# ralexstokes/ethereum_consensus

Hardware: NVIDIA H100
Metric: fast_aggregate_verify tuples/s (higher is better)
Workload: dtype u32 limbs (381-bit Fp), u32 SHA-256 words

## Files before the change

ethereum_consensus_b200/build.py:

```python
from __future__ import annotations

import os
import subprocess
import sys
from concurrent.futures import ThreadPoolExecutor
from pathlib import Path

PKG = Path(__file__).resolve().parent
CSRC = PKG / "csrc"
LIB = PKG / "libb200_consensus.so"
OBJ = PKG / "build"
NVCC = os.environ.get("NVCC", "/usr/local/cuda/bin/nvcc")
ARCH = ["-gencode", "arch=compute_90a,code=sm_90a"]
FLAGS = [*ARCH, "-lineinfo", "-O3", "-std=c++17",
         "-Xcompiler", "-fPIC,-fvisibility=hidden", "--expt-relaxed-constexpr"]
DEFAULT_PTXAS_OPT = {"bls_g1.cu": 2, "bls_g2.cu": 1, "bls_vm.cu": 1}


def _stale(target: Path, deps) -> bool:
    if not target.exists():
        return True
    t = target.stat().st_mtime
    return any(Path(d).stat().st_mtime > t for d in deps)


def build(force: bool = False, verbose: bool = False, defines=(), suffix: str = "", ptxas_opt=None) -> Path:
    global LIB, OBJ
    env_opt = {kv.split(":")[0]: int(kv.split(":")[1]) for kv in os.environ.get("B200_PTXAS_OPT", "").split(",") if kv}
    ptxas_opt = {**DEFAULT_PTXAS_OPT, **env_opt, **dict(ptxas_opt or {})}
    if suffix:
        LIB = PKG / f"libb200_consensus{suffix}.so"
        OBJ = PKG / f"build{suffix}"
    srcs = sorted(CSRC.glob("*.cu"))
    hdrs = sorted(CSRC.glob("*.cuh")) + sorted(CSRC.glob("*.h")) + sorted((PKG.parent / "include").glob("*.h"))
    OBJ.mkdir(exist_ok=True)
    jobs = []
    def command(s, o):
        cmd = [NVCC, *FLAGS, *[f"-D{d}" for d in defines], "-c", str(s), "-o", str(o)]
        if s.name in ptxas_opt and int(ptxas_opt[s.name]) != 3:
            cmd[1:1] = ["-Xptxas", f"-O{int(ptxas_opt[s.name])}"]
        return cmd

    for s in srcs:
        o = OBJ / (s.stem + ".o")
        stamp = o.with_suffix(".cmd")
        if force or _stale(o, [s] + hdrs) or not stamp.exists() or stamp.read_text() != " ".join(command(s, o)):
            jobs.append((s, o))

    def cc(job):
        s, o = job
        cmd = command(s, o)
        stamp = o.with_suffix(".cmd")
        if verbose:
            cmd.insert(1, "-Xptxas=-v")
        r = subprocess.run(cmd, capture_output=True, text=True)
        if r.returncode != 0:
            raise RuntimeError(f"nvcc failed for {s.name}:\n{r.stdout}\n{r.stderr}")
        stamp.write_text(" ".join(command(s, o)))
        return r.stderr

    with ThreadPoolExecutor(max_workers=min(8, max(1, len(jobs)))) as ex:
        for msg in ex.map(cc, jobs):
            if verbose and msg:
                print(msg, file=sys.stderr)
    objs = [OBJ / (s.stem + ".o") for s in srcs]
    if force or jobs or _stale(LIB, objs):
        cmd = [NVCC, "-shared", "-o", str(LIB), *map(str, objs), *ARCH,
               "-Xcompiler", "-fPIC", "-cudart", "static"]
        r = subprocess.run(cmd, capture_output=True, text=True)
        if r.returncode != 0:
            raise RuntimeError(f"link failed:\n{r.stdout}\n{r.stderr}")
    return LIB


if __name__ == "__main__":
    defs = [a[2:] for a in sys.argv[1:] if a.startswith("-D")]
    suf = next((a.split("=", 1)[1] for a in sys.argv[1:] if a.startswith("--suffix=")), "")
    popt = next((a.split("=", 1)[1] for a in sys.argv[1:] if a.startswith("--ptxas-opt=")), "")
    popt = {kv.split(":")[0]: int(kv.split(":")[1]) for kv in popt.split(",") if kv}
    print(build(force="--force" in sys.argv, verbose="-v" in sys.argv, defines=defs, suffix=suf, ptxas_opt=popt))
```

ethereum_consensus_b200/csrc/bls_kernels.cuh:

```cuda
#pragma once
#include <cstddef>
#include <cstdint>

#include "groups.cuh"
#include "fp12.cuh"

namespace b200 {

struct G1Pre {
    Fp xz, y, z3;
    uint32_t inf;
};

enum : uint32_t { TUPLE_FLAG_EMPTY = 1u, TUPLE_FLAG_AGG_INF = 2u };
enum : int32_t { SIG_OK = 0, SIG_NOT_IN_GROUP = -1 };

void set_g1_variant(int v);
void set_g1_small_n(uint32_t n);
void set_small_cta(int threads);
void set_vm_team16_max(uint32_t n);
void set_vm_cta(int threads);
void launch_g1_validate(const uint8_t* keys, uint32_t n, G1Aff* out, int32_t* codes, void* stream, int cta = 0);
void launch_g1_aggregate(const G1Aff* keys, const int32_t* key_codes, const uint32_t* index, const uint32_t* off,
                         uint32_t n_tuples, G1Aff* agg, G1Pre* agg_pre, int32_t* pk_code, uint32_t* flags,
                         uint32_t extra_flags, void* stream, G1Jac* agg_jac = nullptr);
void launch_rlc_scale(const G1Jac* agg, const G2Aff* sig, const int32_t* pk_code, const uint32_t* flags, const int32_t* sig_code,
                      const uint32_t* seed_words, uint64_t t0, uint32_t n, G1Pre* out_g1, G2Jac* out_g2, int32_t* bad, void* stream);
uint32_t launch_rlc_reduce(const Fp12* f_in, const G2Jac* q_in, uint32_t n, Fp12* f_out, G2Jac* q_out, void* stream);
void launch_rlc_finish(const G2Jac* q, G2Aff* out, void* stream);
void launch_fp12_one(Fp12* out, void* stream);
void launch_g2_sig_decode(const uint8_t* sigs, uint32_t n, G2Aff* out, int32_t* sig_code, void* stream);
void launch_hash_to_g2(const uint8_t* msgs, const uint32_t* moff, uint32_t n, G2Aff* out, void* tmp_jac, void* stream);
void launch_miller(const G1Aff* g1, const uint32_t* g1_idx, const G2Aff* g2, const uint32_t* g2_idx,
                   const uint32_t* pair_tuple, const int32_t* pk_code, const uint32_t* flags, const int32_t* sig_code,
                   uint32_t n_pairs, Fp12* f, void* stream);
void launch_final(const Fp12* f, const uint32_t* pair_off, const int32_t* pk_code, const uint32_t* flags,
                  const int32_t* sig_code, uint32_t n_tuples, int32_t* out_codes, void* stream);
int vm_init(void* stream);
int vm_load_programs(const uint32_t* blob, size_t n_words, void* stream);
void launch_vm_miller(const G1Pre* g1, const uint32_t* g1_idx, const G2Aff* g2, const uint32_t* g2_idx,
                      const uint32_t* pair_tuple, const int32_t* pk_code, const uint32_t* flags, const int32_t* sig_code,
                      uint32_t n_pairs, Fp12* f, void* stream);
void launch_vm_final(const Fp12* f, const uint32_t* pair_off, const int32_t* pk_code, const uint32_t* flags,
                     const int32_t* sig_code, uint32_t n_tuples, int32_t* out_codes, void* stream);
void launch_g2_sum_compress(const G2Aff* sigs, const int32_t* sig_code, uint32_t n, uint8_t* out96, int32_t* out_code, void* stream);
void launch_g1_compress(const G1Aff* p, uint8_t* out48, void* stream);
void launch_neg_g1(G1Aff* out, G1Pre* out_pre, void* stream);
void launch_fp_selftest(uint32_t n, uint32_t seed, uint32_t* out_mismatch, void* stream);
enum : int32_t {
    FP_EVAL_MUL = 0, FP_EVAL_SQR = 1, FPL_EVAL_MUL = 2, FPL_EVAL_SQR = 3,
    FP_EVAL_ADD = 4, FP_EVAL_SUB = 5, FP_EVAL_NEG = 6, FPL_EVAL_ADD = 7, FPL_EVAL_SUB = 8, FPL_EVAL_NEG = 9,
    FP_EVAL_ADD_RAW = 10, FP_EVAL_SUB_RAW = 11, FP_EVAL_INV_KALISKI = 12, FP_EVAL_INV_FERMAT = 13,
    FP_EVAL_SQRT = 14, FPL_EVAL_POW_SQRT = 15, FP_EVAL_IS_LEX_LARGEST = 16,
    FP_EVAL_N_OPS = 17,
    FPL_EVAL_SQRT_CHAIN = 18,
    FPL_EVAL_MUL_SUB_MUL = 19, FPL_EVAL_MUL_SUB_8SQR = 20,
    FPL_EVAL_END = 21,
    FP2_EVAL_MUL = 32, FP2_EVAL_SQR = 33, FP2_EVAL_INV = 34, FP2_EVAL_SQRT = 35, FP2_EVAL_SGN0 = 36,
    FP2_EVAL_END = 37
};
constexpr uint32_t kFpEvalIn = 24, kFpEvalOut = 25;
void launch_fp_eval(int32_t op, uint32_t n, const uint32_t* a, const uint32_t* b, uint32_t* out, void* stream);
void launch_fp2_eval(int32_t op, uint32_t n, const uint32_t* a, const uint32_t* b, uint32_t* out, void* stream);
enum : int32_t {
    CURVE_G1L_ADD_MIXED = 0, CURVE_G1L_ADD = 1, CURVE_G1L_IN_SUBGROUP = 2,
    CURVE_G1_N_OPS = 3,
    CURVE_G1L_DOUBLE = 4,
    CURVE_G2_ADD = 32, CURVE_G2_ADD_MIXED = 33, CURVE_G2_DOUBLE = 34, CURVE_G2_IN_SUBGROUP = 35, CURVE_G2_PSI = 36,
    CURVE_G2_CLEAR_COFACTOR = 37, CURVE_G2_SSWU_ISO = 38, CURVE_G2_H2C_FINISH = 39,
    CURVE_G2_END = 40
};
constexpr uint32_t kCurveEvalWords = 73;
void launch_curve_eval(int32_t op, uint32_t n, const uint32_t* a, const uint32_t* b, uint32_t* out, void* stream);
void launch_curve2_eval(int32_t op, uint32_t n, const uint32_t* a, const uint32_t* b, uint32_t* out, void* stream);
enum : int32_t {
    PAIRING_EVAL_FP6_MUL = 0, PAIRING_EVAL_FP6_INV = 1, PAIRING_EVAL_FP12_MUL = 2, PAIRING_EVAL_FP12_SQR = 3,
    PAIRING_EVAL_FP12_INV = 4, PAIRING_EVAL_FP12_MUL_BY_LINE = 5, PAIRING_EVAL_FP12_FROB1 = 6, PAIRING_EVAL_FP12_FROB2 = 7,
    PAIRING_EVAL_FP12_CYCLO_SQR = 8, PAIRING_EVAL_FP12_POW_Z = 9,
    PAIRING_EVAL_MILLER_DOUBLE = 10, PAIRING_EVAL_MILLER_ADD = 11,
    PAIRING_EVAL_MILLER_LOOP = 12, PAIRING_EVAL_FINAL_EXP = 13,
    PAIRING_EVAL_END = 14,
    PAIRING_EVAL_VM_MILLER8 = 32, PAIRING_EVAL_VM_MILLER16 = 33,
    PAIRING_EVAL_VM_FINAL8 = 34, PAIRING_EVAL_VM_FINAL16 = 35,
    PAIRING_EVAL_VM_END = 36,
    PAIRING_EVAL_FOLD_FP12 = 48, PAIRING_EVAL_FOLD_G2 = 49,
    PAIRING_EVAL_FOLD_END = 50
};
constexpr uint32_t kPairingEvalWords = 145;
void launch_pairing_eval(int32_t op, uint32_t n, const uint32_t* a, const uint32_t* b, uint32_t* out, void* stream);
void launch_vm_miller_team(int team, const G1Pre* g1, const uint32_t* idx, const G2Aff* g2, const uint32_t* zeros, uint32_t n,
                           Fp12* f, void* stream);
void launch_vm_final_team(int team, const Fp12* f, const uint32_t* pair_off, const uint32_t* zeros, uint32_t n, Fp12* f_out,
                          int32_t* codes, void* stream);

}
```

ethereum_consensus_b200/csrc/bls_vm.cu:

```cuda
#if defined(B200_VM_MUL_CALL)
#define B200_FP_MUL_CALL 1
#endif
#include <cuda_runtime.h>

#include <algorithm>

#include "bls_kernels.cuh"
#include "pairing_vm.cuh"

namespace b200 {
namespace {

__global__ void k_vm_consts(const uint32_t* __restrict__ plain, Fp2* __restrict__ out) {
    const int i = threadIdx.x;
    if (i < kVmConsts) {
        uint32_t l[24];
        for (int k = 0; k < 24; k++) l[k] = plain[i * 24 + k];
        Fp2 v;
        vm_const_to_mont(v, l);
        out[i] = v;
    }
}

struct VmOuts { int v[6]; };

template <int TEAM>
__device__ __forceinline__ void vm_run(const uint32_t* __restrict__ code, int n_rounds, const Fp2* __restrict__ consts,
                                       const VmRfStrided& rf, uint32_t lane, bool active) {
    uint32_t w = __ldg(code + lane);
#pragma unroll 1
    for (int r = 0; r < n_rounds; r++) {
        const uint32_t w_next = (r + 1 < n_rounds) ? __ldg(code + (r + 1) * TEAM + lane) : 0u;
        if (active && (w & 0xffu) != VM_NOP) {
            Fp2 res;
            vm_exec(w, rf, consts, res);
            rf.store((w >> 8) & 0xffu, res);
        }
        __syncwarp();
        w = w_next;
    }
}

__device__ __forceinline__ bool tuple_dead(uint32_t t, const int32_t* pk_code, const uint32_t* flags, const int32_t* sig_code) {
    return pk_code[t] != BLS_SUCCESS || flags[t] != 0 || sig_code[t] != SIG_OK;
}

template <int TEAM>
__global__ void __launch_bounds__(128) k_vm_miller(const uint32_t* __restrict__ code, const Fp2* __restrict__ consts,
                                                    const G1Pre* __restrict__ g1, const uint32_t* __restrict__ g1_idx,
                                                    const G2Aff* __restrict__ g2, const uint32_t* __restrict__ g2_idx,
                                                    const uint32_t* __restrict__ pair_tuple, const int32_t* __restrict__ pk_code,
                                                    const uint32_t* __restrict__ flags, const int32_t* __restrict__ sig_code,
                                                    uint32_t n_pairs, Fp12* __restrict__ f, int n_rounds, int n_slots, VmOuts outs6) {
    extern __shared__ uint32_t smem[];
    const uint32_t team_in_block = threadIdx.x / TEAM, lane = threadIdx.x % TEAM;
    const uint32_t i = blockIdx.x * (blockDim.x / TEAM) + team_in_block;
    VmRfStrided rf{smem + team_in_block * vm_team_words(uint32_t(n_slots))};
    bool active = i < n_pairs && !tuple_dead(pair_tuple[i], pk_code, flags, sig_code);
    bool trivial = false;
    if (active) {
        const G1Pre* p = g1 + g1_idx[i];
        const G2Aff* q = g2 + g2_idx[i];
        trivial = p->inf || q->inf;
        if (!trivial) {
            if (lane == 0) { Fp2 v; v.c0 = p->xz; v.c1 = fp_zero(); rf.store(0, v); }
            if (lane == 1) { Fp2 v; v.c0 = p->y; v.c1 = fp_zero(); rf.store(1, v); }
            if (lane == 2) { Fp2 v; v.c0 = p->z3; v.c1 = fp_zero(); rf.store(2, v); }
            if (lane == 3) rf.store(3, q->x);
            if (lane == 4) rf.store(4, q->y);
        }
    }
    __syncwarp();
    vm_run<TEAM>(code, n_rounds, consts, rf, lane, active && !trivial);
    static_assert(TEAM >= 6, "team must cover the six output coefficients");
    if (active && lane < 6) {
        Fp2 v;
        if (trivial) v = (lane == 0) ? fp2_one() : fp2_zero();
        else v = rf.load(uint32_t(outs6.v[lane]));
        Fp2* dst = reinterpret_cast<Fp2*>(f + i);
        const int tower_pos[6] = {0, 3, 1, 4, 2, 5};
        dst[tower_pos[lane]] = v;
    }
}

template <int TEAM, bool STORE = false>
__global__ void __launch_bounds__(128) k_vm_final(const uint32_t* __restrict__ code, const Fp2* __restrict__ consts,
                                                  const Fp12* __restrict__ f, const uint32_t* __restrict__ pair_off,
                                                  const int32_t* __restrict__ pk_code, const uint32_t* __restrict__ flags,
                                                  const int32_t* __restrict__ sig_code, uint32_t n_tuples,
                                                  int32_t* __restrict__ out_codes, int n_rounds, int n_slots, VmOuts outs6,
                                                  Fp12* __restrict__ f_out = nullptr) {
    extern __shared__ uint32_t smem[];
    const uint32_t team_in_block = threadIdx.x / TEAM, lane = threadIdx.x % TEAM;
    const uint32_t t = blockIdx.x * (blockDim.x / TEAM) + team_in_block;
    VmRfStrided rf{smem + team_in_block * vm_team_words(uint32_t(n_slots))};
    int32_t code_out = BLS_SUCCESS;
    bool active = false;
    if (t < n_tuples) {
        if (pk_code[t] != BLS_SUCCESS) code_out = pk_code[t];
        else if (sig_code[t] > 0) code_out = sig_code[t];
        else if (flags[t] != 0 || sig_code[t] == SIG_NOT_IN_GROUP) code_out = BLS_VERIFY_FAIL;
        else active = true;
    }
    if (active) {
        const int tower_pos[6] = {0, 3, 1, 4, 2, 5};
        for (uint32_t k = lane; k < 12; k += TEAM) {
            const Fp2* src = reinterpret_cast<const Fp2*>(f + pair_off[t] + k / 6);
            rf.store(k, src[tower_pos[k % 6]]);
        }
    }
    __syncwarp();
    vm_run<TEAM>(code, n_rounds, consts, rf, lane, active);
    if (STORE && active && lane < 6) {
        const int tower_pos[6] = {0, 3, 1, 4, 2, 5};
        reinterpret_cast<Fp2*>(f_out + t)[tower_pos[lane]] = rf.load(uint32_t(outs6.v[lane]));
    }
    if (t < n_tuples && lane == 0) {
        if (active) {
            bool one = fp2_eq(rf.load(uint32_t(outs6.v[0])), fp2_one());
#pragma unroll 1
            for (int k = 1; k < 6; k++) one = one && fp2_is_zero(rf.load(uint32_t(outs6.v[k])));
            code_out = one ? BLS_SUCCESS : BLS_VERIFY_FAIL;
        }
        out_codes[t] = code_out;
    }
}

}

struct VmProgramDev {
    uint32_t* d_code = nullptr;
    int rounds = 0, slots = 0;
    VmOuts outs{};
};
static VmProgramDev g_miller_prog[2], g_final_prog[2];
static Fp2* g_d_consts = nullptr;
static uint32_t g_team16_max = 2048;
static int g_vm_cta = 32;
void set_vm_team16_max(uint32_t n) { g_team16_max = n; }
void set_vm_cta(int threads) { if (threads == 32 || threads == 64 || threads == 128) g_vm_cta = threads; }

static int vm_set_program(VmProgramDev& p, const uint32_t* code, size_t bytes, int rounds, int slots, const int* outs, cudaStream_t st) {
    uint32_t* d = nullptr;
    if (cudaMalloc(&d, bytes) != cudaSuccess) return 1;
    if (cudaMemcpyAsync(d, code, bytes, cudaMemcpyHostToDevice, st) != cudaSuccess) return 1;
    if (cudaStreamSynchronize(st) != cudaSuccess) return 1;
    if (p.d_code) cudaFree(p.d_code);
    p.d_code = d; p.rounds = rounds; p.slots = slots;
    for (int k = 0; k < 6; k++) p.outs.v[k] = outs[k];
    return 0;
}
template <int TEAM>
static int vm_upload(int slot, cudaStream_t st) {
    typedef VmProg<TEAM> P;
    if (vm_set_program(g_miller_prog[slot], P::miller_code(), P::miller_code_bytes, P::miller_rounds, P::miller_slots, P::miller_out, st)) return 1;
    if (vm_set_program(g_final_prog[slot], P::final_code(), P::final_code_bytes, P::final_rounds, P::final_slots, P::final_out, st)) return 1;
    cudaFuncSetAttribute(k_vm_miller<TEAM>, cudaFuncAttributeMaxDynamicSharedMemorySize, kVmMaxSmemBytes);
    cudaFuncSetAttribute(k_vm_final<TEAM>, cudaFuncAttributeMaxDynamicSharedMemorySize, kVmMaxSmemBytes);
    cudaFuncSetAttribute(k_vm_final<TEAM, true>, cudaFuncAttributeMaxDynamicSharedMemorySize, kVmMaxSmemBytes);
    return 0;
}

int vm_load_programs(const uint32_t* blob, size_t n_words, void* stream) {
    if (!blob || n_words < 18 || blob[0] != kVmBlobMagic) return 1;
    const uint32_t team = blob[1], mr = blob[2], ms = blob[3], fr = blob[10], fs = blob[11];
    if (team != 8 && team != 16) return 1;
    if (!mr || !fr || mr > (1u << 20) || fr > (1u << 20) || ms < 12 || fs < 12 || ms > 255 || fs > 255) return 1;
    if (n_words != 18 + size_t(mr) * team + size_t(fr) * team) return 1;
    if (size_t(32 / team) * vm_team_words(std::max(ms, fs)) * 4 > size_t(kVmMaxSmemBytes)) return 1;
    auto check = [&](const uint32_t* code, uint32_t rounds, uint32_t slots, const uint32_t* outs) {
        for (int k = 0; k < 6; k++) if (outs[k] >= slots) return false;
        for (size_t i = 0; i < size_t(rounds) * team; i++) {
            const uint32_t w = code[i], op = w & 0xffu, d = (w >> 8) & 0xffu, a = (w >> 16) & 0xffu, b = w >> 24;
            if (op > VM_LDC) return false;
            if (op == VM_NOP) continue;
            if (d >= slots) return false;
            if (op == VM_LDC) { if (a >= uint32_t(kVmConsts)) return false; continue; }
            if (a >= slots) return false;
            const bool binary = op == VM_MUL || op == VM_MULFP || op == VM_ADD || op == VM_SUB;
            if (binary && b >= slots) return false;
        }
        return true;
    };
    const uint32_t* mcode = blob + 18;
    const uint32_t* fcode = mcode + size_t(mr) * team;
    if (!check(mcode, mr, ms, blob + 4) || !check(fcode, fr, fs, blob + 12)) return 1;
    int mo[6], fo[6];
    for (int k = 0; k < 6; k++) { mo[k] = int(blob[4 + k]); fo[k] = int(blob[12 + k]); }
    cudaStream_t st = static_cast<cudaStream_t>(stream);
    const int slot = team == 8 ? 0 : 1;
    if (vm_set_program(g_miller_prog[slot], mcode, size_t(mr) * team * 4, int(mr), int(ms), mo, st)) return 1;
    if (vm_set_program(g_final_prog[slot], fcode, size_t(fr) * team * 4, int(fr), int(fs), fo, st)) return 1;
    return 0;
}

int vm_init(void* stream) {
    if (g_d_consts) return 0;
    cudaStream_t st = static_cast<cudaStream_t>(stream);
    uint32_t* d_plain = nullptr;
    if (vm_upload<8>(0, st) || vm_upload<16>(1, st)) return 1;
    if (cudaMalloc(&g_d_consts, sizeof(Fp2) * kVmConsts) != cudaSuccess) return 1;
    if (cudaMalloc(&d_plain, sizeof(h_vm_consts)) != cudaSuccess) return 1;
    cudaMemcpyAsync(d_plain, h_vm_consts, sizeof(h_vm_consts), cudaMemcpyHostToDevice, st);
    k_vm_consts<<<1, 32, 0, st>>>(d_plain, g_d_consts);
    if (cudaStreamSynchronize(st) != cudaSuccess) return 1;
    cudaFree(d_plain);
    return cudaGetLastError() == cudaSuccess ? 0 : 1;
}

template <int TEAM>
static void launch_vm_miller_t(int slot, const G1Pre* g1, const uint32_t* g1_idx, const G2Aff* g2, const uint32_t* g2_idx,
                               const uint32_t* pair_tuple, const int32_t* pk_code, const uint32_t* flags, const int32_t* sig_code,
                               uint32_t n_pairs, Fp12* f, cudaStream_t st) {
    const VmProgramDev& p = g_miller_prog[slot];
    int threads = g_vm_cta;
    while (threads > 32 && size_t(threads / TEAM) * vm_team_words(uint32_t(p.slots)) * 4 > size_t(kVmMaxSmemBytes)) threads >>= 1;
    const int teams = threads / TEAM;
    const size_t smem = size_t(teams) * vm_team_words(uint32_t(p.slots)) * 4;
    k_vm_miller<TEAM><<<(n_pairs + teams - 1) / teams, threads, smem, st>>>(
        p.d_code, g_d_consts, g1, g1_idx, g2, g2_idx, pair_tuple, pk_code, flags, sig_code, n_pairs, f, p.rounds, p.slots, p.outs);
}
template <int TEAM, bool STORE = false>
static void launch_vm_final_t(int slot, const Fp12* f, const uint32_t* pair_off, const int32_t* pk_code, const uint32_t* flags,
                              const int32_t* sig_code, uint32_t n_tuples, int32_t* out_codes, cudaStream_t st,
                              Fp12* f_out = nullptr) {
    const VmProgramDev& p = g_final_prog[slot];
    int threads = g_vm_cta;
    while (threads > 32 && size_t(threads / TEAM) * vm_team_words(uint32_t(p.slots)) * 4 > size_t(kVmMaxSmemBytes)) threads >>= 1;
    const int teams = threads / TEAM;
    const size_t smem = size_t(teams) * vm_team_words(uint32_t(p.slots)) * 4;
    k_vm_final<TEAM, STORE><<<(n_tuples + teams - 1) / teams, threads, smem, st>>>(
        p.d_code, g_d_consts, f, pair_off, pk_code, flags, sig_code, n_tuples, out_codes, p.rounds, p.slots, p.outs, f_out);
}

void launch_vm_miller(const G1Pre* g1, const uint32_t* g1_idx, const G2Aff* g2, const uint32_t* g2_idx,
                      const uint32_t* pair_tuple, const int32_t* pk_code, const uint32_t* flags, const int32_t* sig_code,
                      uint32_t n_pairs, Fp12* f, void* stream) {
    if (!n_pairs) return;
    cudaStream_t st = static_cast<cudaStream_t>(stream);
    if (n_pairs <= g_team16_max) launch_vm_miller_t<16>(1, g1, g1_idx, g2, g2_idx, pair_tuple, pk_code, flags, sig_code, n_pairs, f, st);
    else launch_vm_miller_t<8>(0, g1, g1_idx, g2, g2_idx, pair_tuple, pk_code, flags, sig_code, n_pairs, f, st);
}
void launch_vm_final(const Fp12* f, const uint32_t* pair_off, const int32_t* pk_code, const uint32_t* flags,
                     const int32_t* sig_code, uint32_t n_tuples, int32_t* out_codes, void* stream) {
    if (!n_tuples) return;
    cudaStream_t st = static_cast<cudaStream_t>(stream);
    if (n_tuples <= g_team16_max) launch_vm_final_t<16>(1, f, pair_off, pk_code, flags, sig_code, n_tuples, out_codes, st);
    else launch_vm_final_t<8>(0, f, pair_off, pk_code, flags, sig_code, n_tuples, out_codes, st);
}

void launch_vm_miller_team(int team, const G1Pre* g1, const uint32_t* idx, const G2Aff* g2, const uint32_t* zeros, uint32_t n,
                           Fp12* f, void* stream) {
    if (!n) return;
    cudaStream_t st = static_cast<cudaStream_t>(stream);
    const int32_t* z = reinterpret_cast<const int32_t*>(zeros);
    if (team == 16) launch_vm_miller_t<16>(1, g1, idx, g2, idx, zeros, z, zeros, z, n, f, st);
    else launch_vm_miller_t<8>(0, g1, idx, g2, idx, zeros, z, zeros, z, n, f, st);
}
void launch_vm_final_team(int team, const Fp12* f, const uint32_t* pair_off, const uint32_t* zeros, uint32_t n, Fp12* f_out,
                          int32_t* codes, void* stream) {
    if (!n) return;
    cudaStream_t st = static_cast<cudaStream_t>(stream);
    const int32_t* z = reinterpret_cast<const int32_t*>(zeros);
    if (team == 16) launch_vm_final_t<16, true>(1, f, pair_off, z, zeros, z, n, codes, st, f_out);
    else launch_vm_final_t<8, true>(0, f, pair_off, z, zeros, z, n, codes, st, f_out);
}

}
```

ethereum_consensus_b200/csrc/capi_bls.cu:

```cuda
#include <algorithm>
#include <cctype>
#include <cstdlib>
#include <cstring>
#include <memory>
#include <random>
#include <string>
#include <type_traits>
#include <vector>

#include "bls_kernels.cuh"
#include "comm.h"
#include "engine.h"

namespace b200 {

struct BlsState {
    cudaStream_t sb = nullptr, sc = nullptr;
    static constexpr uint32_t kMaxChunks = 16;
    cudaStream_t sd = nullptr, se = nullptr;
    cudaEvent_t ev_ck[kMaxChunks] = {nullptr}, ev_join = nullptr;
    uint32_t chunks = 1, chunk_min_tuples = 2048;
    int chunk_k1_cta = 128;
    bool chunk_alt = true;
    bool key_split = true;
    int k1_first_cta = 128;
    cudaEvent_t ev_in = nullptr, ev_b = nullptr, ev_c = nullptr, ev_k0 = nullptr, ev_k1 = nullptr, ev_d0 = nullptr, ev_d1 = nullptr;
    DevBuf keys, key_aff, key_code, g1pts, g1pre, pk_code, flags, sigs, g2pts, sig_code, msgs, small, f, out, h2c_tmp, gath;
    DevBuf rlc_jac, rlc_g1, rlc_q, rlc_fa, rlc_fb, rlc_qa, rlc_qb, rlc_zero, rlc_idx, rlc_misc, rlc_xch;
    PinnedBuf stage;
    G1Aff* d_negg1 = nullptr;
    G1Pre* d_negg1_pre = nullptr;
    DevBuf reg_aff, reg_code;
    size_t reg_n = 0;
    float last_dominant_ms = 0.f;
    bool trace = false;
    cudaEvent_t ev_t[8] = {nullptr};
    int small_order = 0;
    int small_cta_override = 0;
    bool use_vm = true;

    ~BlsState() {
        for (cudaStream_t st : {sb, sc, sd, se}) if (st) cudaStreamDestroy(st);
        for (cudaEvent_t ev : ev_ck) if (ev) cudaEventDestroy(ev);
        for (cudaEvent_t ev : ev_t) if (ev) cudaEventDestroy(ev);
        for (cudaEvent_t ev : {ev_join, ev_in, ev_b, ev_c, ev_k0, ev_k1, ev_d0, ev_d1}) if (ev) cudaEventDestroy(ev);
        cudaFree(d_negg1);
        cudaFree(d_negg1_pre);
    }
};

struct Knob {
    const char* name;
    void (*set)(BlsState&, int64_t);
};
static const Knob kKnobs[] = {
    {"bls_chunks", [](BlsState& s, int64_t v) { s.chunks = uint32_t(std::max<int64_t>(1, v)); }},
    {"bls_chunk_min_tuples", [](BlsState& s, int64_t v) { s.chunk_min_tuples = uint32_t(std::max<int64_t>(2, v)); }},
    {"bls_chunk_k1_cta", [](BlsState& s, int64_t v) { s.chunk_k1_cta = int(v); }},
    {"bls_chunk_alt", [](BlsState& s, int64_t v) { s.chunk_alt = v != 0; }},
    {"bls_key_split", [](BlsState& s, int64_t v) { s.key_split = v != 0; }},
    {"bls_k1_first_cta", [](BlsState& s, int64_t v) { s.k1_first_cta = (v == 128) ? 128 : 384; }},
    {"bls_small_cta", [](BlsState& s, int64_t v) { s.small_cta_override = int(v); }},
    {"vm_team16_max", [](BlsState&, int64_t v) { set_vm_team16_max(uint32_t(std::max<int64_t>(0, v))); }},
    {"vm_cta", [](BlsState&, int64_t v) { set_vm_cta(int(v)); }},
};

static void read_env(BlsState& s, int* side_prio, int* pair_prio) {
    for (const Knob& k : kKnobs) {
        std::string var = "B200_";
        for (const char* c = k.name; *c; c++) var += char(toupper(static_cast<unsigned char>(*c)));
        if (const char* v = getenv(var.c_str())) k.set(s, atoll(v));
    }
    if (const char* v = getenv("B200_G1_VARIANT")) set_g1_variant(atoi(v));
    if (const char* v = getenv("B200_G1_SMALL_N")) set_g1_small_n(uint32_t(atol(v)));
    if (const char* v = getenv("B200_PAIRING_VM")) s.use_vm = atoi(v) != 0;
    if (const char* v = getenv("B200_BLS_TRACE")) s.trace = atoi(v) != 0;
    if (const char* v = getenv("B200_SMALL_ORDER")) s.small_order = atoi(v);
    if (const char* v = getenv("B200_SMALL_STREAM_PRIORITY")) *side_prio = atoi(v);
    *pair_prio = *side_prio;
    if (const char* v = getenv("B200_PAIR_STREAM_PRIORITY")) *pair_prio = atoi(v);
}

static int32_t bls_state(Engine& e, BlsState** out) {
    if (!e.bls) {
        std::unique_ptr<BlsState> s(new BlsState());
        for (auto& ev : s->ev_t) B200_CUDA_TRY(cudaEventCreate(&ev));
        int prio_lo = 0, prio = 0, prio_d = 0;
        B200_CUDA_TRY(cudaDeviceGetStreamPriorityRange(&prio_lo, &prio));
        read_env(*s, &prio, &prio_d);
        B200_CUDA_TRY(cudaStreamCreateWithPriority(&s->sb, cudaStreamNonBlocking, prio));
        B200_CUDA_TRY(cudaStreamCreateWithPriority(&s->sc, cudaStreamNonBlocking, prio));
        B200_CUDA_TRY(cudaStreamCreateWithPriority(&s->sd, cudaStreamNonBlocking, prio_d));
        B200_CUDA_TRY(cudaStreamCreateWithPriority(&s->se, cudaStreamNonBlocking, prio_lo));
        for (auto& ev : s->ev_ck) B200_CUDA_TRY(cudaEventCreateWithFlags(&ev, cudaEventDisableTiming));
        B200_CUDA_TRY(cudaEventCreateWithFlags(&s->ev_join, cudaEventDisableTiming));
        B200_CUDA_TRY(cudaEventCreateWithFlags(&s->ev_c, cudaEventDisableTiming));
        B200_CUDA_TRY(cudaEventCreateWithFlags(&s->ev_in, cudaEventDisableTiming));
        B200_CUDA_TRY(cudaEventCreateWithFlags(&s->ev_b, cudaEventDisableTiming));
        B200_CUDA_TRY(cudaEventCreate(&s->ev_k0));
        B200_CUDA_TRY(cudaEventCreate(&s->ev_k1));
        B200_CUDA_TRY(cudaEventCreate(&s->ev_d0));
        B200_CUDA_TRY(cudaEventCreate(&s->ev_d1));
        B200_CUDA_TRY(cudaMalloc(&s->d_negg1, sizeof(G1Aff)));
        B200_CUDA_TRY(cudaMalloc(&s->d_negg1_pre, sizeof(G1Pre)));
        launch_neg_g1(s->d_negg1, s->d_negg1_pre, e.stream);
        e.launches++;
        if (vm_init(e.stream) != 0) { e.last_error = "pairing VM initialisation failed"; return B200_ERR_CUDA; }
        e.launches++;
        B200_CUDA_TRY(cudaGetLastError());
        B200_CUDA_TRY(cudaStreamSynchronize(e.stream));
        e.bls = s.release();
    }
    *out = static_cast<BlsState*>(e.bls);
    return B200_SUCCESS;
}

enum PairMode { MODE_FAST_AGGREGATE = 0, MODE_AGGREGATE = 1 };
constexpr size_t kMaxBatchTuples = size_t(1) << 26;
constexpr size_t kRegistryExtraKeys = size_t(1) << 16;
constexpr size_t kRlcPart = sizeof(Fp12) + sizeof(G2Jac) + 16;

struct RlcReq {
    const uint8_t* seed32;
    uint64_t t0;
    bool exchange;
    int32_t all_ok;
};

struct Batch {
    PairMode mode = MODE_FAST_AGGREGATE;
    const uint8_t* keys = nullptr;
    uint32_t n_keys = 0;
    const uint32_t* index = nullptr;
    uint32_t n_index = 0;
    const uint32_t* key_off = nullptr;
    const uint8_t* msgs = nullptr;
    const uint32_t* msg_off = nullptr;
    uint32_t n_msgs = 0;
    const uint8_t* sigs = nullptr;
    uint32_t T = 0;
    bool force_fail_shape = false;
    RlcReq* rlc = nullptr;
};

struct VerifyRun {
    Engine& e;
    BlsState& s;
    const Batch& b;
    const uint32_t T = b.T, n_keys = b.n_keys, n_msgs = b.n_msgs;
    const bool fa = b.mode == MODE_FAST_AGGREGATE, registry = b.index != nullptr;
    const uint32_t n_g1 = (fa ? T : n_keys) + 1;
    const uint32_t n_pairs = fa ? 2 * T : (b.force_fail_shape ? 0 : n_msgs + 1);
    const uint32_t n_g2 = n_msgs + T;
    const uint32_t msg_bytes = b.msg_off[n_msgs];
    const uint32_t rlc_world = b.rlc && b.rlc->exchange ? uint32_t(comm().world) : 1u;
    const cudaStream_t sa = e.stream;
    size_t o_koff = 0, o_index = 0, o_moff = 0;
    const uint32_t *d_small = nullptr, *d_g1i = nullptr, *d_g2i = nullptr, *d_ptu = nullptr, *d_poff = nullptr;
    int32_t* h_out = nullptr;
    bool chunked = false;

    int32_t run(int32_t* out_codes);
    int32_t reserve_buffers();
    int32_t stage_small();
    int32_t key_phase();
    int32_t keys_chunked(uint32_t n_chunks);
    int32_t keys_one_range(uint32_t k_split);
    int32_t launch_small();
    void pairing_tail();
    int32_t rlc_tail();
    int32_t readback(void* h_dst, const void* d_src, size_t bytes);
};

int32_t VerifyRun::run(int32_t* out_codes) {
    if (b.rlc && (!fa || !s.use_vm)) return B200_ERR_BAD_ARG;
    int32_t rc;
    if ((rc = reserve_buffers()) || (rc = stage_small()) || (rc = key_phase())) return rc;
    if (b.rlc) return rlc_tail();
    if (!chunked) pairing_tail();
    if ((rc = readback(h_out + 4, s.out.p, size_t(T) * 4))) return rc;
    if (s.trace) {
        float a = 0, b1 = 0, c = 0, d = 0, f2 = 0, g2 = 0;
        cudaEventElapsedTime(&a, s.ev_k0, s.ev_d0); cudaEventElapsedTime(&b1, s.ev_t[0], s.ev_t[1]);
        cudaEventElapsedTime(&c, s.ev_t[1], s.ev_t[2]); cudaEventElapsedTime(&d, s.ev_t[2], s.ev_t[3]);
        cudaEventElapsedTime(&f2, s.ev_t[3], s.ev_k1); cudaEventElapsedTime(&g2, s.ev_k0, s.ev_k1);
        fprintf(stderr, "[b200 bls] pre-K1 %.2f | K1 %.2f | K2 %.2f | wait(streamB) %.2f | miller %.2f | final %.2f | total %.2f ms\n",
                a, s.last_dominant_ms, b1, c, d, f2, g2);
    }
    for (uint32_t t = 0; t < T; t++) out_codes[t] = h_out[4 + t];
    return B200_SUCCESS;
}

int32_t VerifyRun::reserve_buffers() {
    B200_CUDA_TRY(s.keys.reserve(size_t(n_keys) * 48 + 64));
    B200_CUDA_TRY(s.key_aff.reserve(size_t(n_keys + 1) * sizeof(G1Aff)));
    B200_CUDA_TRY(s.key_code.reserve(size_t(n_keys + 1) * 4));
    B200_CUDA_TRY(s.g1pts.reserve(size_t(n_g1) * sizeof(G1Aff)));
    B200_CUDA_TRY(s.g1pre.reserve(size_t(n_g1) * sizeof(G1Pre)));
    B200_CUDA_TRY(s.pk_code.reserve(size_t(T + 1) * 4));
    B200_CUDA_TRY(s.flags.reserve(size_t(T + 1) * 4));
    B200_CUDA_TRY(s.sigs.reserve(size_t(T) * 96 + 64));
    B200_CUDA_TRY(s.g2pts.reserve(size_t(n_g2 + 1) * sizeof(G2Aff)));
    B200_CUDA_TRY(s.sig_code.reserve(size_t(T + 1) * 4));
    B200_CUDA_TRY(s.msgs.reserve(size_t(msg_bytes) + 64));
    B200_CUDA_TRY(s.f.reserve(size_t(n_pairs + 1) * sizeof(Fp12)));
    B200_CUDA_TRY(s.out.reserve(size_t(T + 1) * 4));
    B200_CUDA_TRY(s.h2c_tmp.reserve(size_t(2 * n_msgs + 2) * sizeof(G2Jac)));
    if (!b.rlc) return B200_SUCCESS;
    const uint32_t rlc_part = (T + 31) / 32 + rlc_world + 2;
    B200_CUDA_TRY(s.rlc_jac.reserve(size_t(T + 1) * sizeof(G1Jac)));
    B200_CUDA_TRY(s.rlc_g1.reserve(size_t(T + 2) * sizeof(G1Pre)));
    B200_CUDA_TRY(s.rlc_q.reserve(size_t(T + 1) * sizeof(G2Jac)));
    B200_CUDA_TRY(s.rlc_fa.reserve(size_t(rlc_part) * sizeof(Fp12)));
    B200_CUDA_TRY(s.rlc_fb.reserve(size_t(rlc_part) * sizeof(Fp12)));
    B200_CUDA_TRY(s.rlc_qa.reserve(size_t(rlc_part) * sizeof(G2Jac)));
    B200_CUDA_TRY(s.rlc_qb.reserve(size_t(rlc_part) * sizeof(G2Jac)));
    B200_CUDA_TRY(s.rlc_zero.reserve(size_t(T + 8) * 4));
    B200_CUDA_TRY(s.rlc_idx.reserve(size_t(2 * (T + 1)) * 4));
    B200_CUDA_TRY(s.rlc_misc.reserve(256));
    B200_CUDA_TRY(s.rlc_xch.reserve(size_t(rlc_world + 1) * kRlcPart));
    return B200_SUCCESS;
}

int32_t VerifyRun::stage_small() {
    const uint32_t n_koff = fa ? T + 1 : 2;
    std::vector<uint32_t> small;
    small.reserve(size_t(n_koff) + b.n_index + n_msgs + 1 + 3 * size_t(n_pairs) + T + 1 + 8);
    o_koff = small.size();
    if (fa) small.insert(small.end(), b.key_off, b.key_off + T + 1);
    else { small.push_back(0); small.push_back(n_keys); }
    o_index = small.size();
    if (registry) small.insert(small.end(), b.index, b.index + b.n_index);
    o_moff = small.size();
    small.insert(small.end(), b.msg_off, b.msg_off + n_msgs + 1);
    const size_t o_g1i = small.size();
    small.resize(small.size() + 3 * size_t(n_pairs) + T + 1);
    uint32_t* g1i = small.data() + o_g1i;
    uint32_t* g2i = g1i + n_pairs;
    uint32_t* ptu = g2i + n_pairs;
    uint32_t* poff = ptu + n_pairs;
    if (fa) {
        for (uint32_t t = 0; t < T; t++) {
            g1i[2 * t] = t;          g2i[2 * t] = t;
            g1i[2 * t + 1] = T;      g2i[2 * t + 1] = n_msgs + t;
            ptu[2 * t] = ptu[2 * t + 1] = t;
            poff[t] = 2 * t;
        }
        poff[T] = 2 * T;
    } else {
        for (uint32_t i = 0; i + 1 < n_pairs; i++) { g1i[i] = i; g2i[i] = i; ptu[i] = 0; }
        if (n_pairs) { g1i[n_pairs - 1] = n_keys; g2i[n_pairs - 1] = n_msgs; ptu[n_pairs - 1] = 0; }
        poff[0] = 0; poff[1] = n_pairs;
    }
    const size_t small_bytes = small.size() * 4;
    B200_CUDA_TRY(s.stage.reserve(small_bytes + size_t(T + 1) * 4 + 64 +
                                  (b.rlc ? 256 + size_t(rlc_world) * kRlcPart + size_t(8 + 2 * (T + 1)) * 4 : 0)));
    B200_CUDA_TRY(s.small.reserve(small_bytes + 64));
    memcpy(s.stage.p, small.data(), small_bytes);
    h_out = reinterpret_cast<int32_t*>(static_cast<uint8_t*>(s.stage.p) + ((small_bytes + 15) & ~size_t(15)));
    d_small = static_cast<const uint32_t*>(s.small.p);
    d_g1i = d_small + o_g1i;
    d_g2i = d_g1i + n_pairs;
    d_ptu = d_g2i + n_pairs;
    d_poff = d_ptu + n_pairs;
    B200_CUDA_TRY(cudaMemcpyAsync(s.small.p, s.stage.p, small_bytes, cudaMemcpyHostToDevice, sa));
    B200_CUDA_TRY(cudaEventRecord(s.ev_in, sa));
    return B200_SUCCESS;
}

int32_t VerifyRun::key_phase() {
    const bool have_k1 = n_keys != 0;
    const uint32_t n_chunks = (fa && !b.rlc && s.use_vm && have_k1 && !registry && s.small_order == 0 && !b.force_fail_shape &&
                               s.chunks > 1 && T >= s.chunk_min_tuples) ? std::min(s.chunks, BlsState::kMaxChunks) : 1u;
    constexpr uint32_t kSplitWaves = 4, kSplitKeys = kSplitWaves * 148u * 384u;
    const uint32_t k_split = (s.key_split && have_k1 && !registry && n_chunks == 1 && s.small_order == 0 && n_keys >= 4u * kSplitKeys)
                                 ? kSplitKeys : n_keys;
    if (n_keys) B200_CUDA_TRY(cudaMemcpyAsync(s.keys.p, b.keys, size_t(k_split) * 48, cudaMemcpyHostToDevice, sa));
    B200_CUDA_TRY(cudaEventRecord(s.ev_k0, sa));
    set_small_cta(s.small_cta_override ? s.small_cta_override : ((have_k1 && n_keys >= 148u * 384u && s.small_order == 0 && T > 1024) ? 128 : 32));
    if (have_k1 && s.small_order == 1) {
        int32_t rc = launch_small();
        if (rc) return rc;
        B200_CUDA_TRY(cudaStreamWaitEvent(sa, s.ev_b, 0));
        B200_CUDA_TRY(cudaStreamWaitEvent(sa, s.ev_c, 0));
    }
    B200_CUDA_TRY(cudaEventRecord(s.ev_d0, sa));
    chunked = n_chunks > 1;
    return chunked ? keys_chunked(n_chunks) : keys_one_range(k_split);
}

int32_t VerifyRun::keys_chunked(uint32_t n_chunks) {
    cudaStream_t sd = s.sd;
    uint32_t tb[BlsState::kMaxChunks + 1];
    for (uint32_t c = 0; c <= n_chunks; c++) tb[c] = uint32_t(uint64_t(T) * c / n_chunks);
    B200_CUDA_TRY(cudaStreamWaitEvent(s.se, s.ev_k0, 0));
    for (uint32_t c = 0; c < n_chunks; c++) {
        const uint32_t k0 = b.key_off[tb[c]], k1 = b.key_off[tb[c + 1]];
        cudaStream_t sk = ((c & 1u) && s.chunk_alt) ? s.se : sa;
        launch_g1_validate(static_cast<const uint8_t*>(s.keys.p) + size_t(k0) * 48, k1 - k0, static_cast<G1Aff*>(s.key_aff.p) + k0,
                           static_cast<int32_t*>(s.key_code.p) + k0, sk, s.chunk_k1_cta);
        if (k1 > k0) e.launches++;
        B200_CUDA_TRY(cudaEventRecord(s.ev_ck[c], sk));
        if (c == 0) {
            int32_t rc = launch_small();
            if (rc) return rc;
        }
    }
    if (s.chunk_alt)
        for (uint32_t c = 1; c < n_chunks; c += 2) B200_CUDA_TRY(cudaStreamWaitEvent(sa, s.ev_ck[c], 0));
    B200_CUDA_TRY(cudaEventRecord(s.ev_d1, sa));
    B200_CUDA_TRY(cudaStreamWaitEvent(sd, s.ev_in, 0));
    B200_CUDA_TRY(cudaStreamWaitEvent(sd, s.ev_b, 0));
    B200_CUDA_TRY(cudaStreamWaitEvent(sd, s.ev_c, 0));
    B200_CUDA_TRY(cudaMemcpyAsync(static_cast<G1Pre*>(s.g1pre.p) + T, s.d_negg1_pre, sizeof(G1Pre), cudaMemcpyDeviceToDevice, sd));
    int32_t* d_pk = static_cast<int32_t*>(s.pk_code.p);
    uint32_t* d_fl = static_cast<uint32_t*>(s.flags.p);
    const int32_t* d_sc = static_cast<const int32_t*>(s.sig_code.p);
    for (uint32_t c = 0; c < n_chunks; c++) {
        const uint32_t t0 = tb[c], nt = tb[c + 1] - tb[c];
        if (!nt) continue;
        B200_CUDA_TRY(cudaStreamWaitEvent(sd, s.ev_ck[c], 0));
        launch_g1_aggregate(static_cast<const G1Aff*>(s.key_aff.p), static_cast<const int32_t*>(s.key_code.p), nullptr, d_small + o_koff + t0,
                            nt, nullptr, static_cast<G1Pre*>(s.g1pre.p) + t0, d_pk + t0, d_fl + t0, 0u, sd, nullptr);
        launch_vm_miller(static_cast<const G1Pre*>(s.g1pre.p), d_g1i + 2 * t0, static_cast<const G2Aff*>(s.g2pts.p), d_g2i + 2 * t0,
                         d_ptu + 2 * t0, d_pk, d_fl, d_sc, 2 * nt, static_cast<Fp12*>(s.f.p) + 2 * size_t(t0), sd);
        launch_vm_final(static_cast<const Fp12*>(s.f.p), d_poff + t0, d_pk + t0, d_fl + t0, d_sc + t0, nt,
                        static_cast<int32_t*>(s.out.p) + t0, sd);
        e.launches += 3;
    }
    B200_CUDA_TRY(cudaEventRecord(s.ev_join, sd));
    B200_CUDA_TRY(cudaStreamWaitEvent(sa, s.ev_join, 0));
    if (s.trace) { cudaEventRecord(s.ev_t[0], sa); cudaEventRecord(s.ev_t[1], sa); cudaEventRecord(s.ev_t[2], sa); cudaEventRecord(s.ev_t[3], sa); }
    return B200_SUCCESS;
}

int32_t VerifyRun::keys_one_range(uint32_t k_split) {
    const bool have_k1 = n_keys != 0;
    G1Aff* d_g1 = static_cast<G1Aff*>(s.g1pts.p);
    const G1Aff* key_aff = registry ? static_cast<const G1Aff*>(s.reg_aff.p) : static_cast<const G1Aff*>(s.key_aff.p);
    const int32_t* key_code = registry ? static_cast<const int32_t*>(s.reg_code.p) : static_cast<const int32_t*>(s.key_code.p);
    G1Aff* k1_aff = registry ? static_cast<G1Aff*>(s.reg_aff.p) + s.reg_n : static_cast<G1Aff*>(s.key_aff.p);
    int32_t* k1_code = registry ? static_cast<int32_t*>(s.reg_code.p) + s.reg_n : static_cast<int32_t*>(s.key_code.p);
    if (have_k1) {
        launch_g1_validate(static_cast<const uint8_t*>(s.keys.p), k_split, k1_aff, k1_code, sa, k_split < n_keys ? s.k1_first_cta : 0);
        e.launches++;
    }
    if (!(have_k1 && s.small_order == 1)) {
        if (have_k1 && s.small_order == 2) {
            B200_CUDA_TRY(cudaEventRecord(s.ev_in, sa));
        }
        int32_t rc = launch_small();
        if (rc) return rc;
    }
    if (k_split < n_keys) {
        B200_CUDA_TRY(cudaStreamWaitEvent(s.se, s.ev_k0, 0));
        B200_CUDA_TRY(cudaMemcpyAsync(static_cast<uint8_t*>(s.keys.p) + size_t(k_split) * 48, b.keys + size_t(k_split) * 48,
                                      size_t(n_keys - k_split) * 48, cudaMemcpyHostToDevice, s.se));
        launch_g1_validate(static_cast<const uint8_t*>(s.keys.p) + size_t(k_split) * 48, n_keys - k_split, k1_aff + k_split,
                           k1_code + k_split, s.se, 384);
        e.launches++;
        B200_CUDA_TRY(cudaEventRecord(s.ev_ck[0], s.se));
        B200_CUDA_TRY(cudaStreamWaitEvent(sa, s.ev_ck[0], 0));
    }
    B200_CUDA_TRY(cudaEventRecord(s.ev_d1, sa));
    if (s.trace) cudaEventRecord(s.ev_t[0], sa);
    launch_g1_aggregate(key_aff, key_code, registry ? d_small + o_index : nullptr, d_small + o_koff, fa ? T : 1,
                        (fa && !s.use_vm) ? d_g1 : nullptr, (fa && s.use_vm) ? static_cast<G1Pre*>(s.g1pre.p) : nullptr,
                        static_cast<int32_t*>(s.pk_code.p), static_cast<uint32_t*>(s.flags.p),
                        b.force_fail_shape ? uint32_t(TUPLE_FLAG_EMPTY) : 0u, sa, b.rlc ? static_cast<G1Jac*>(s.rlc_jac.p) : nullptr);
    e.launches++;
    if (fa) {
        B200_CUDA_TRY(cudaMemcpyAsync(d_g1 + T, s.d_negg1, sizeof(G1Aff), cudaMemcpyDeviceToDevice, sa));
        B200_CUDA_TRY(cudaMemcpyAsync(static_cast<G1Pre*>(s.g1pre.p) + T, s.d_negg1_pre, sizeof(G1Pre), cudaMemcpyDeviceToDevice, sa));
    } else {
        B200_CUDA_TRY(cudaMemcpyAsync(static_cast<G1Aff*>(s.key_aff.p) + n_keys, s.d_negg1, sizeof(G1Aff), cudaMemcpyDeviceToDevice, sa));
    }
    if (s.trace) cudaEventRecord(s.ev_t[1], sa);
    B200_CUDA_TRY(cudaStreamWaitEvent(sa, s.ev_b, 0));
    B200_CUDA_TRY(cudaStreamWaitEvent(sa, s.ev_c, 0));
    if (s.trace) cudaEventRecord(s.ev_t[2], sa);
    return B200_SUCCESS;
}

int32_t VerifyRun::launch_small() {
    cudaStream_t sb = s.sb, sc = s.sc;
    B200_CUDA_TRY(cudaStreamWaitEvent(sb, s.ev_in, 0));
    B200_CUDA_TRY(cudaStreamWaitEvent(sc, s.ev_in, 0));
    if (T) B200_CUDA_TRY(cudaMemcpyAsync(s.sigs.p, b.sigs, size_t(T) * 96, cudaMemcpyHostToDevice, sb));
    if (msg_bytes) B200_CUDA_TRY(cudaMemcpyAsync(s.msgs.p, b.msgs, msg_bytes, cudaMemcpyHostToDevice, sc));
    launch_g2_sig_decode(static_cast<const uint8_t*>(s.sigs.p), T, static_cast<G2Aff*>(s.g2pts.p) + n_msgs, static_cast<int32_t*>(s.sig_code.p), sb);
    launch_hash_to_g2(static_cast<const uint8_t*>(s.msgs.p), d_small + o_moff, n_msgs, static_cast<G2Aff*>(s.g2pts.p), s.h2c_tmp.p, sc);
    e.launches += (T ? 1 : 0) + (n_msgs ? 2 : 0);
    B200_CUDA_TRY(cudaEventRecord(s.ev_b, sb));
    B200_CUDA_TRY(cudaEventRecord(s.ev_c, sc));
    return B200_SUCCESS;
}

void VerifyRun::pairing_tail() {
    const G2Aff* d_g2 = static_cast<const G2Aff*>(s.g2pts.p);
    const int32_t* d_pk = static_cast<const int32_t*>(s.pk_code.p);
    const uint32_t* d_fl = static_cast<const uint32_t*>(s.flags.p);
    const int32_t* d_sc = static_cast<const int32_t*>(s.sig_code.p);
    if (fa && s.use_vm) {
        launch_vm_miller(static_cast<const G1Pre*>(s.g1pre.p), d_g1i, d_g2, d_g2i, d_ptu, d_pk, d_fl, d_sc, n_pairs, static_cast<Fp12*>(s.f.p), sa);
        if (s.trace) cudaEventRecord(s.ev_t[3], sa);
        launch_vm_final(static_cast<const Fp12*>(s.f.p), d_poff, d_pk, d_fl, d_sc, T, static_cast<int32_t*>(s.out.p), sa);
    } else {
        const G1Aff* pair_g1 = static_cast<const G1Aff*>(fa ? s.g1pts.p : s.key_aff.p);
        launch_miller(pair_g1, d_g1i, d_g2, d_g2i, d_ptu, d_pk, d_fl, d_sc, n_pairs, static_cast<Fp12*>(s.f.p), sa);
        launch_final(static_cast<const Fp12*>(s.f.p), d_poff, d_pk, d_fl, d_sc, T, static_cast<int32_t*>(s.out.p), sa);
    }
    e.launches += (n_pairs ? 1 : 0) + (T ? 1 : 0);
}

int32_t VerifyRun::readback(void* h_dst, const void* d_src, size_t bytes) {
    B200_CUDA_TRY(cudaEventRecord(s.ev_k1, sa));
    B200_CUDA_TRY(cudaGetLastError());
    B200_CUDA_TRY(cudaMemcpyAsync(h_dst, d_src, bytes, cudaMemcpyDeviceToHost, sa));
    B200_CUDA_TRY(cudaStreamSynchronize(sa));
    B200_CUDA_TRY(cudaStreamSynchronize(s.sb));
    B200_CUDA_TRY(cudaStreamSynchronize(s.sc));
    if (chunked) B200_CUDA_TRY(cudaStreamSynchronize(s.sd));
    B200_CUDA_TRY(cudaEventElapsedTime(&e.last_kernel_ms, s.ev_k0, s.ev_k1));
    B200_CUDA_TRY(cudaEventElapsedTime(&s.last_dominant_ms, s.ev_d0, s.ev_d1));
    return B200_SUCCESS;
}

template <class T>
static const T* rlc_fold(Engine& e, const T* in, uint32_t n, T* const buf[2], int& pp, cudaStream_t st) {
    do {
        if constexpr (std::is_same_v<T, Fp12>) n = launch_rlc_reduce(in, nullptr, n, buf[pp], nullptr, st);
        else n = launch_rlc_reduce(nullptr, in, n, nullptr, buf[pp], st);
        e.launches++;
        in = buf[pp]; pp ^= 1;
    } while (n > 1);
    return in;
}

int32_t VerifyRun::rlc_tail() {
    RlcReq* rlc = b.rlc;
    G2Aff* d_g2 = static_cast<G2Aff*>(s.g2pts.p);
    const size_t kPart = kRlcPart;
    uint8_t* h_x = reinterpret_cast<uint8_t*>(h_out + 16);
    uint32_t* d_zero = static_cast<uint32_t*>(s.rlc_zero.p);
    uint32_t* d_idx = static_cast<uint32_t*>(s.rlc_idx.p);
    uint8_t* d_misc = static_cast<uint8_t*>(s.rlc_misc.p);
    G1Pre* d_rg1 = static_cast<G1Pre*>(s.rlc_g1.p);
    G2Jac* d_rq = static_cast<G2Jac*>(s.rlc_q.p);
    B200_CUDA_TRY(cudaMemsetAsync(d_zero, 0, size_t(T + 8) * 4, sa));
    B200_CUDA_TRY(cudaMemsetAsync(d_misc + 32, 0, 96, sa));
    {
        uint32_t* h = reinterpret_cast<uint32_t*>(h_x + ((size_t(rlc_world) * kPart + 63) & ~size_t(63)));
        for (int i = 0; i < 8; i++)
            h[i] = (uint32_t(rlc->seed32[4 * i]) << 24) | (uint32_t(rlc->seed32[4 * i + 1]) << 16) | (uint32_t(rlc->seed32[4 * i + 2]) << 8) | rlc->seed32[4 * i + 3];
        uint32_t* hi = h + 8;
        for (uint32_t t = 0; t <= T; t++) { hi[t] = t; hi[T + 1 + t] = t < T ? t : n_g2; }
        B200_CUDA_TRY(cudaMemcpyAsync(d_misc, h, 32, cudaMemcpyHostToDevice, sa));
        B200_CUDA_TRY(cudaMemcpyAsync(d_idx, hi, size_t(2 * (T + 1)) * 4, cudaMemcpyHostToDevice, sa));
    }
    launch_rlc_scale(static_cast<const G1Jac*>(s.rlc_jac.p), d_g2 + n_msgs, static_cast<const int32_t*>(s.pk_code.p),
                     static_cast<const uint32_t*>(s.flags.p), static_cast<const int32_t*>(s.sig_code.p),
                     reinterpret_cast<const uint32_t*>(d_misc), rlc->t0, T, d_rg1, d_rq, reinterpret_cast<int32_t*>(d_misc + 32), sa);
    B200_CUDA_TRY(cudaMemcpyAsync(d_rg1 + T, s.d_negg1_pre, sizeof(G1Pre), cudaMemcpyDeviceToDevice, sa));
    if (s.trace) cudaEventRecord(s.ev_t[3], sa);
    Fp12* fbuf[2] = {static_cast<Fp12*>(s.rlc_fa.p), static_cast<Fp12*>(s.rlc_fb.p)};
    G2Jac* qbuf[2] = {static_cast<G2Jac*>(s.rlc_qa.p), static_cast<G2Jac*>(s.rlc_qb.p)};
    int pp = 0;
    const G2Jac* qi = rlc_fold(e, d_rq, T, qbuf, pp, sa);
    launch_rlc_finish(qi, d_g2 + n_g2, sa);
    launch_vm_miller(d_rg1, d_idx, d_g2, d_idx + T + 1, d_zero, reinterpret_cast<const int32_t*>(d_zero), d_zero,
                     reinterpret_cast<const int32_t*>(d_zero), T + 1, static_cast<Fp12*>(s.f.p), sa);
    pp = 0;
    const Fp12* fi = rlc_fold(e, static_cast<const Fp12*>(s.f.p), T + 1, fbuf, pp, sa);
    if (rlc->exchange && rlc_world > 1) {
        uint8_t* x = static_cast<uint8_t*>(s.rlc_xch.p);
        B200_CUDA_TRY(cudaMemcpyAsync(x, fi, sizeof(Fp12), cudaMemcpyDeviceToDevice, sa));
        B200_CUDA_TRY(cudaMemcpyAsync(x + sizeof(Fp12) + sizeof(G2Jac), d_misc + 32, 16, cudaMemcpyDeviceToDevice, sa));
        int32_t rcx = comm_all_gather(e, x, x + kPart, kPart, sa);
        if (rcx) return rcx;
        for (uint32_t r = 0; r < rlc_world; r++)
            B200_CUDA_TRY(cudaMemcpyAsync(fbuf[pp] + r, x + kPart * (1 + r), sizeof(Fp12), cudaMemcpyDeviceToDevice, sa));
        B200_CUDA_TRY(cudaMemcpyAsync(h_x, x + kPart, size_t(rlc_world) * kPart, cudaMemcpyDeviceToHost, sa));
        fi = fbuf[pp]; pp ^= 1;
        fi = rlc_fold(e, fi, rlc_world, fbuf, pp, sa);
    }
    Fp12* d_fin = fbuf[pp];
    B200_CUDA_TRY(cudaMemcpyAsync(d_fin, fi, sizeof(Fp12), cudaMemcpyDeviceToDevice, sa));
    launch_fp12_one(d_fin + 1, sa);
    launch_vm_final(d_fin, d_zero, reinterpret_cast<const int32_t*>(d_zero), d_zero, reinterpret_cast<const int32_t*>(d_zero), 1,
                    reinterpret_cast<int32_t*>(d_misc + 64), sa);
    e.launches += 5;
    int32_t rc = readback(h_out, d_misc + 32, 64);
    if (rc) return rc;
    bool bad = h_out[0] != 0;
    if (rlc->exchange && rlc_world > 1)
        for (uint32_t r = 0; r < rlc_world; r++) {
            int32_t flag;
            memcpy(&flag, h_x + size_t(r) * kPart + sizeof(Fp12) + sizeof(G2Jac), 4);
            bad = bad || flag != 0;
        }
    rlc->all_ok = (!bad && h_out[8] == BLS_SUCCESS) ? 1 : 0;
    if (s.trace) {
        float a = 0, g2 = 0;
        cudaEventElapsedTime(&a, s.ev_t[2], s.ev_k1); cudaEventElapsedTime(&g2, s.ev_k0, s.ev_k1);
        fprintf(stderr, "[b200 bls rlc] K1 %.2f | scale + T Miller loops + folds + 1 final exponentiation %.2f | total %.2f ms\n",
                s.last_dominant_ms, a, g2);
    }
    return B200_SUCCESS;
}

static int32_t run_verify(Engine& e, BlsState& s, const Batch& b, int32_t* out_codes) {
    const int32_t rc = VerifyRun{e, s, b}.run(out_codes);
    if (rc != B200_SUCCESS) {
        cudaStreamSynchronize(e.stream);
        cudaStreamSynchronize(s.sb);
        cudaStreamSynchronize(s.sc);
        cudaStreamSynchronize(s.sd);
        cudaStreamSynchronize(s.se);
        cudaGetLastError();
    }
    return rc;
}


static int32_t check_offsets(const uint32_t* off, size_t n_tuples, uint32_t* count) {
    for (size_t t = 0; t < n_tuples; t++)
        if (off[t] > off[t + 1]) return B200_ERR_BAD_ARG;
    *count = off[n_tuples];
    return B200_SUCCESS;
}

static std::vector<uint32_t> msg32_offsets(size_t n_tuples) {
    std::vector<uint32_t> moff(n_tuples + 1);
    for (size_t t = 0; t <= n_tuples; t++) moff[t] = uint32_t(32 * t);
    return moff;
}

struct TupleRange {
    size_t lo, cnt;
};
static TupleRange tuple_shard(size_t n_tuples, size_t world, size_t rank) {
    const size_t base = n_tuples / world, rem = n_tuples % world;
    return {rank * base + std::min(rank, rem), base + (rank < rem ? 1 : 0)};
}

static Batch shard_batch(const uint8_t* pks_flat, const uint32_t* pk_offsets, const uint8_t* msgs32, const uint8_t* sigs, TupleRange r,
                         std::vector<uint32_t>& koff, std::vector<uint32_t>& moff) {
    koff.resize(r.cnt + 1);
    for (size_t t = 0; t <= r.cnt; t++) koff[t] = pk_offsets[r.lo + t] - pk_offsets[r.lo];
    moff = msg32_offsets(r.cnt);
    return {.keys = pks_flat ? pks_flat + size_t(pk_offsets[r.lo]) * 48 : nullptr, .n_keys = koff[r.cnt], .key_off = koff.data(),
            .msgs = msgs32 + 32 * r.lo, .msg_off = moff.data(), .n_msgs = uint32_t(r.cnt), .sigs = sigs + 96 * r.lo, .T = uint32_t(r.cnt)};
}

static int32_t check_indices(Engine& e, const BlsState& s, const uint32_t* index, uint32_t n, size_t n_extra) {
    for (uint32_t i = 0; i < n; i++)
        if (index[i] >= s.reg_n + n_extra) {
            e.last_error = n_extra ? "validator index outside the loaded registry (+ extra keys)" : "validator index outside the loaded registry";
            return B200_ERR_BAD_ARG;
        }
    return B200_SUCCESS;
}

static void rlc_seed(const uint8_t* seed32, uint8_t out[32]) {
    if (seed32) { memcpy(out, seed32, 32); return; }
    std::random_device rd;
    for (int i = 0; i < 8; i++) { const uint32_t v = rd(); memcpy(out + 4 * i, &v, 4); }
}

static int32_t verify_all(Engine& e, BlsState& s, Batch b, const uint8_t* seed32, uint64_t t0, bool exchange, int32_t* all_ok) {
    uint8_t seed[32];
    rlc_seed(seed32, seed);
    RlcReq req{seed, t0, exchange, 0};
    b.rlc = &req;
    const int32_t rc = run_verify(e, s, b, nullptr);
    if (rc) return rc;
    *all_ok = req.all_ok;
    return B200_SUCCESS;
}

}

using namespace b200;

extern "C" {

int32_t b200_tune(const char* knob, int64_t value) {
    Engine& e = engine();
    Guard g(e);
    int32_t rc = check_ready(e);
    if (rc) return rc;
    BlsState* s;
    rc = bls_state(e, &s);
    if (rc) return rc;
    if (!knob) return B200_ERR_BAD_ARG;
    for (const Knob& k : kKnobs)
        if (strcmp(k.name, knob) == 0) { k.set(*s, value); return B200_SUCCESS; }
    return B200_ERR_BAD_ARG;
}

int32_t b200_vm_load_programs(const uint32_t* blob, size_t n_words) {
    Engine& e = engine();
    Guard g(e);
    int32_t rc = check_ready(e);
    if (rc) return rc;
    BlsState* s;
    rc = bls_state(e, &s);
    if (rc) return rc;
    B200_CUDA_TRY(cudaStreamSynchronize(e.stream));
    if (vm_load_programs(blob, n_words, e.stream) != 0) { e.last_error = "malformed pairing-VM program blob"; return B200_ERR_BAD_ARG; }
    return B200_SUCCESS;
}

float b200_last_dominant_kernel_ms(void) {
    Engine& e = engine();
    return e.bls ? static_cast<BlsState*>(e.bls)->last_dominant_ms : 0.f;
}

int32_t b200_fp_selftest(uint32_t n, uint32_t seed, uint32_t* mismatches) {
    Engine& e = engine();
    Guard g(e);
    int32_t rc = check_ready(e);
    if (rc) return rc;
    if (!mismatches) return B200_ERR_BAD_ARG;
    uint32_t* d = nullptr;
    B200_CUDA_TRY(cudaMalloc(&d, 4));
    B200_CUDA_TRY(cudaMemsetAsync(d, 0, 4, e.stream));
    launch_fp_selftest(n, seed, d, e.stream);
    e.launches++;
    B200_CUDA_TRY(cudaGetLastError());
    B200_CUDA_TRY(cudaMemcpyAsync(mismatches, d, 4, cudaMemcpyDeviceToHost, e.stream));
    B200_CUDA_TRY(cudaStreamSynchronize(e.stream));
    cudaFree(d);
    return B200_SUCCESS;
}

int32_t b200_fp_eval(int32_t op, uint32_t n, const uint32_t* a, const uint32_t* b, uint32_t* out) {
    Engine& e = engine();
    Guard g(e);
    int32_t rc = check_ready(e);
    if (rc) return rc;
    const bool fp2 = op >= FP2_EVAL_MUL && op < FP2_EVAL_END;
    if (!(fp2 || (op >= 0 && op < FP_EVAL_N_OPS) || (op >= FPL_EVAL_SQRT_CHAIN && op < FPL_EVAL_END)) || n > (1u << 24))
        return B200_ERR_BAD_ARG;
    if (n == 0) return B200_SUCCESS;
    if (!a || !b || !out) return B200_ERR_BAD_ARG;
    const size_t in_bytes = size_t(n) * kFpEvalIn * 4, out_bytes = size_t(n) * kFpEvalOut * 4;
    uint32_t* d = nullptr;
    B200_CUDA_TRY(cudaMalloc(&d, 2 * in_bytes + out_bytes));
    uint32_t* da = d;
    uint32_t* db = d + size_t(n) * kFpEvalIn;
    uint32_t* dout = db + size_t(n) * kFpEvalIn;
    cudaMemcpyAsync(da, a, in_bytes, cudaMemcpyHostToDevice, e.stream);
    cudaMemcpyAsync(db, b, in_bytes, cudaMemcpyHostToDevice, e.stream);
    if (fp2) launch_fp2_eval(op, n, da, db, dout, e.stream);
    else launch_fp_eval(op, n, da, db, dout, e.stream);
    e.launches++;
    cudaError_t ce = cudaGetLastError();
    if (ce == cudaSuccess) ce = cudaMemcpyAsync(out, dout, out_bytes, cudaMemcpyDeviceToHost, e.stream);
    if (ce == cudaSuccess) ce = cudaStreamSynchronize(e.stream);
    cudaFree(d);
    if (ce != cudaSuccess) { e.last_error = cudaGetErrorString(ce); return B200_ERR_CUDA; }
    return B200_SUCCESS;
}

int32_t b200_curve_eval(int32_t op, uint32_t n, const uint32_t* a, const uint32_t* b, uint32_t* out) {
    Engine& e = engine();
    Guard g(e);
    int32_t rc = check_ready(e);
    if (rc) return rc;
    const bool g2 = op >= CURVE_G2_ADD && op < CURVE_G2_END;
    if (!(g2 || (op >= 0 && op < CURVE_G1_N_OPS) || op == CURVE_G1L_DOUBLE) || n > (1u << 24)) return B200_ERR_BAD_ARG;
    if (n == 0) return B200_SUCCESS;
    if (!a || !b || !out) return B200_ERR_BAD_ARG;
    const size_t bytes = size_t(n) * kCurveEvalWords * 4;
    uint32_t* d = nullptr;
    B200_CUDA_TRY(cudaMalloc(&d, 3 * bytes));
    uint32_t* da = d;
    uint32_t* db = d + size_t(n) * kCurveEvalWords;
    uint32_t* dout = db + size_t(n) * kCurveEvalWords;
    cudaMemcpyAsync(da, a, bytes, cudaMemcpyHostToDevice, e.stream);
    cudaMemcpyAsync(db, b, bytes, cudaMemcpyHostToDevice, e.stream);
    if (g2) launch_curve2_eval(op, n, da, db, dout, e.stream);
    else launch_curve_eval(op, n, da, db, dout, e.stream);
    e.launches++;
    cudaError_t ce = cudaGetLastError();
    if (ce == cudaSuccess) ce = cudaMemcpyAsync(out, dout, bytes, cudaMemcpyDeviceToHost, e.stream);
    if (ce == cudaSuccess) ce = cudaStreamSynchronize(e.stream);
    cudaFree(d);
    if (ce != cudaSuccess) { e.last_error = cudaGetErrorString(ce); return B200_ERR_CUDA; }
    return B200_SUCCESS;
}

int32_t b200_pairing_eval(int32_t op, uint32_t n, const uint32_t* a, const uint32_t* b, uint32_t* out) {
    Engine& e = engine();
    Guard g(e);
    int32_t rc = check_ready(e);
    if (rc) return rc;
    const bool vm = op >= PAIRING_EVAL_VM_MILLER8 && op < PAIRING_EVAL_VM_END;
    const bool fold = op >= PAIRING_EVAL_FOLD_FP12 && op < PAIRING_EVAL_FOLD_END;
    if (!(vm || fold || (op >= 0 && op < PAIRING_EVAL_END)) || n > (1u << 24)) return B200_ERR_BAD_ARG;
    if (n == 0) return B200_SUCCESS;
    if (!a || !b || !out) return B200_ERR_BAD_ARG;
    BlsState* s;
    if ((rc = bls_state(e, &s))) return rc;
    constexpr size_t W = kPairingEvalWords;
    const size_t rec_bytes = size_t(n) * W * 4;
    cudaStream_t st = e.stream;
    std::vector<uint32_t> h_out(size_t(n) * W, 0);
    const int team = (op == PAIRING_EVAL_VM_MILLER16 || op == PAIRING_EVAL_VM_FINAL16) ? 16 : 8;
    uint8_t* d = nullptr;
    const size_t scratch = 3 * rec_bytes + size_t(n) * (sizeof(Fp12) * 3 + sizeof(G2Jac) + sizeof(G1Pre) + sizeof(G2Aff) + 12) + 4096;
    B200_CUDA_TRY(cudaMalloc(&d, scratch));
    auto carve = [&, off = size_t(0)](size_t bytes) mutable { uint8_t* p = d + off; off += (bytes + 255) & ~size_t(255); return p; };
    auto fp12_of = [&](const uint32_t* rec) { Fp12 v; memcpy(&v, rec, sizeof(Fp12)); return v; };
    auto put = [&](size_t i, const void* v, size_t bytes, uint32_t flag) {
        memcpy(&h_out[i * W], v, bytes);
        h_out[i * W + 144] = flag;
    };
    static_assert(sizeof(Fp12) == 144 * 4 && sizeof(G2Jac) == 72 * 4, "records hold the structs' words in order");
    cudaError_t ce = cudaSuccess;
    if (!vm && !fold) {
        uint32_t* da = reinterpret_cast<uint32_t*>(carve(rec_bytes));
        uint32_t* db = reinterpret_cast<uint32_t*>(carve(rec_bytes));
        uint32_t* dout = reinterpret_cast<uint32_t*>(carve(rec_bytes));
        cudaMemcpyAsync(da, a, rec_bytes, cudaMemcpyHostToDevice, st);
        cudaMemcpyAsync(db, b, rec_bytes, cudaMemcpyHostToDevice, st);
        launch_pairing_eval(op, n, da, db, dout, st);
        e.launches++;
        ce = cudaGetLastError();
        if (ce == cudaSuccess) ce = cudaMemcpyAsync(h_out.data(), dout, rec_bytes, cudaMemcpyDeviceToHost, st);
        if (ce == cudaSuccess) ce = cudaStreamSynchronize(st);
    } else if (op == PAIRING_EVAL_VM_MILLER8 || op == PAIRING_EVAL_VM_MILLER16) {
        std::vector<G1Pre> g1(n);
        std::vector<G2Aff> g2(n);
        std::vector<uint32_t> idx(n);
        for (uint32_t i = 0; i < n; i++) {
            memcpy(&g1[i], a + i * W, 3 * sizeof(Fp)); g1[i].inf = a[i * W + 144];
            memcpy(&g2[i], b + i * W, 2 * sizeof(Fp2)); g2[i].inf = b[i * W + 144];
            idx[i] = i;
        }
        G1Pre* dg1 = reinterpret_cast<G1Pre*>(carve(n * sizeof(G1Pre)));
        G2Aff* dg2 = reinterpret_cast<G2Aff*>(carve(n * sizeof(G2Aff)));
        uint32_t* didx = reinterpret_cast<uint32_t*>(carve(n * 4));
        uint32_t* dzero = reinterpret_cast<uint32_t*>(carve(n * 4));
        Fp12* df = reinterpret_cast<Fp12*>(carve(n * sizeof(Fp12)));
        std::vector<Fp12> f(n);
        cudaMemcpyAsync(dg1, g1.data(), n * sizeof(G1Pre), cudaMemcpyHostToDevice, st);
        cudaMemcpyAsync(dg2, g2.data(), n * sizeof(G2Aff), cudaMemcpyHostToDevice, st);
        cudaMemcpyAsync(didx, idx.data(), n * 4, cudaMemcpyHostToDevice, st);
        cudaMemsetAsync(dzero, 0, n * 4, st);
        launch_vm_miller_team(team, dg1, didx, dg2, dzero, n, df, st);
        e.launches++;
        ce = cudaGetLastError();
        if (ce == cudaSuccess) ce = cudaMemcpyAsync(f.data(), df, n * sizeof(Fp12), cudaMemcpyDeviceToHost, st);
        if (ce == cudaSuccess) ce = cudaStreamSynchronize(st);
        for (uint32_t i = 0; i < n; i++) put(i, &f[i], sizeof(Fp12), 0);
    } else if (vm) {
        std::vector<Fp12> f(2 * size_t(n));
        std::vector<uint32_t> off(n);
        for (uint32_t i = 0; i < n; i++) { f[2 * i] = fp12_of(a + i * W); f[2 * i + 1] = fp12_of(b + i * W); off[i] = 2 * i; }
        Fp12* df = reinterpret_cast<Fp12*>(carve(2 * n * sizeof(Fp12)));
        Fp12* dfo = reinterpret_cast<Fp12*>(carve(n * sizeof(Fp12)));
        uint32_t* doff = reinterpret_cast<uint32_t*>(carve(n * 4));
        uint32_t* dzero = reinterpret_cast<uint32_t*>(carve(n * 4));
        int32_t* dcodes = reinterpret_cast<int32_t*>(carve(n * 4));
        std::vector<Fp12> fo(n);
        std::vector<int32_t> codes(n);
        cudaMemcpyAsync(df, f.data(), 2 * n * sizeof(Fp12), cudaMemcpyHostToDevice, st);
        cudaMemcpyAsync(doff, off.data(), n * 4, cudaMemcpyHostToDevice, st);
        cudaMemsetAsync(dzero, 0, n * 4, st);
        launch_vm_final_team(team, df, doff, dzero, n, dfo, dcodes, st);
        e.launches++;
        ce = cudaGetLastError();
        if (ce == cudaSuccess) ce = cudaMemcpyAsync(fo.data(), dfo, n * sizeof(Fp12), cudaMemcpyDeviceToHost, st);
        if (ce == cudaSuccess) ce = cudaMemcpyAsync(codes.data(), dcodes, n * 4, cudaMemcpyDeviceToHost, st);
        if (ce == cudaSuccess) ce = cudaStreamSynchronize(st);
        for (uint32_t i = 0; i < n; i++) put(i, &fo[i], sizeof(Fp12), codes[i] == BLS_SUCCESS ? 1u : 0u);
    } else if (op == PAIRING_EVAL_FOLD_FP12) {
        std::vector<Fp12> f(n);
        for (uint32_t i = 0; i < n; i++) f[i] = fp12_of(a + i * W);
        Fp12* df = reinterpret_cast<Fp12*>(carve(n * sizeof(Fp12)));
        Fp12* buf[2] = {reinterpret_cast<Fp12*>(carve(n * sizeof(Fp12))), reinterpret_cast<Fp12*>(carve(n * sizeof(Fp12)))};
        cudaMemcpyAsync(df, f.data(), n * sizeof(Fp12), cudaMemcpyHostToDevice, st);
        int pp = 0;
        const Fp12* r = rlc_fold(e, static_cast<const Fp12*>(df), n, buf, pp, st);
        Fp12 v;
        ce = cudaGetLastError();
        if (ce == cudaSuccess) ce = cudaMemcpyAsync(&v, r, sizeof(Fp12), cudaMemcpyDeviceToHost, st);
        if (ce == cudaSuccess) ce = cudaStreamSynchronize(st);
        put(0, &v, sizeof(Fp12), 0);
    } else {
        std::vector<G2Jac> q(n);
        for (uint32_t i = 0; i < n; i++) memcpy(&q[i], a + i * W, sizeof(G2Jac));
        G2Jac* dq = reinterpret_cast<G2Jac*>(carve(n * sizeof(G2Jac)));
        G2Jac* buf[2] = {reinterpret_cast<G2Jac*>(carve(n * sizeof(G2Jac))), reinterpret_cast<G2Jac*>(carve(n * sizeof(G2Jac)))};
        G2Aff* daff = reinterpret_cast<G2Aff*>(carve(sizeof(G2Aff)));
        cudaMemcpyAsync(dq, q.data(), n * sizeof(G2Jac), cudaMemcpyHostToDevice, st);
        int pp = 0;
        launch_rlc_finish(rlc_fold(e, static_cast<const G2Jac*>(dq), n, buf, pp, st), daff, st);
        e.launches++;
        G2Aff v;
        ce = cudaGetLastError();
        if (ce == cudaSuccess) ce = cudaMemcpyAsync(&v, daff, sizeof(G2Aff), cudaMemcpyDeviceToHost, st);
        if (ce == cudaSuccess) ce = cudaStreamSynchronize(st);
        put(0, &v, 2 * sizeof(Fp2), v.inf);
    }
    cudaFree(d);
    if (ce != cudaSuccess) { e.last_error = cudaGetErrorString(ce); return B200_ERR_CUDA; }
    memcpy(out, h_out.data(), rec_bytes);
    return B200_SUCCESS;
}

int32_t b200_fast_aggregate_verify_batch(const uint8_t* pks_flat, const uint32_t* pk_offsets, const uint8_t* msgs32,
                                         const uint8_t* sigs, size_t n_tuples, int32_t* out_codes) {
    Engine& e = engine();
    Guard g(e);
    int32_t rc = check_ready(e);
    if (rc) return rc;
    if (n_tuples == 0) return B200_SUCCESS;
    if (!pk_offsets || !msgs32 || !sigs || !out_codes || n_tuples > kMaxBatchTuples) return B200_ERR_BAD_ARG;
    uint32_t nk;
    if ((rc = check_offsets(pk_offsets, n_tuples, &nk))) return rc;
    if (nk && !pks_flat) return B200_ERR_BAD_ARG;
    BlsState* s;
    rc = bls_state(e, &s);
    if (rc) return rc;
    const std::vector<uint32_t> moff = msg32_offsets(n_tuples);
    return run_verify(e, *s, {.keys = pks_flat, .n_keys = nk, .key_off = pk_offsets, .msgs = msgs32, .msg_off = moff.data(),
                              .n_msgs = uint32_t(n_tuples), .sigs = sigs, .T = uint32_t(n_tuples)}, out_codes);
}

int32_t b200_fast_aggregate_verify_batch_sharded(const uint8_t* pks_flat, const uint32_t* pk_offsets, const uint8_t* msgs32,
                                                 const uint8_t* sigs, size_t n_tuples, int32_t* out_codes) {
    Engine& e = engine();
    Guard g(e);
    int32_t rc = check_ready(e);
    if (rc) return rc;
    const Comm& c = comm();
    if (!c.ready) { e.last_error = "b200_comm_init has not been called"; return B200_ERR_NOT_INITIALIZED; }
    if (n_tuples == 0) return B200_SUCCESS;
    if (!pk_offsets || !msgs32 || !sigs || !out_codes || n_tuples > kMaxBatchTuples) return B200_ERR_BAD_ARG;
    uint32_t nk;
    if ((rc = check_offsets(pk_offsets, n_tuples, &nk))) return rc;
    if (nk && !pks_flat) return B200_ERR_BAD_ARG;
    BlsState* s;
    rc = bls_state(e, &s);
    if (rc) return rc;
    const size_t world = size_t(c.world);
    const TupleRange mine = tuple_shard(n_tuples, world, size_t(c.rank));
    const size_t per = (n_tuples + world - 1) / world;
    B200_CUDA_TRY(s->out.reserve((per + 1) * 4));
    B200_CUDA_TRY(s->gath.reserve(world * per * 4 + 16));
    if (mine.cnt) {
        std::vector<uint32_t> koff, moff;
        std::vector<int32_t> local(mine.cnt);
        rc = run_verify(e, *s, shard_batch(pks_flat, pk_offsets, msgs32, sigs, mine, koff, moff), local.data());
        if (rc) return rc;
    }
    cudaStream_t sa = e.stream;
    int32_t* d_out = static_cast<int32_t*>(s->out.p);
    if (per > mine.cnt) B200_CUDA_TRY(cudaMemsetAsync(d_out + mine.cnt, 0xff, (per - mine.cnt) * 4, sa));
    rc = comm_all_gather(e, d_out, s->gath.p, per * 4, sa);
    if (rc) return rc;
    B200_CUDA_TRY(s->stage.reserve(world * per * 4 + 64));
    B200_CUDA_TRY(cudaMemcpyAsync(s->stage.p, s->gath.p, world * per * 4, cudaMemcpyDeviceToHost, sa));
    B200_CUDA_TRY(cudaStreamSynchronize(sa));
    const int32_t* h = static_cast<const int32_t*>(s->stage.p);
    for (size_t r = 0; r < world; r++) {
        const TupleRange theirs = tuple_shard(n_tuples, world, r);
        memcpy(out_codes + theirs.lo, h + r * per, theirs.cnt * 4);
    }
    return B200_SUCCESS;
}

int32_t b200_fast_aggregate_verify_batch_all(const uint8_t* pks_flat, const uint32_t* pk_offsets, const uint8_t* msgs32,
                                             const uint8_t* sigs, size_t n_tuples, const uint8_t* seed32, int32_t* all_ok) {
    Engine& e = engine();
    Guard g(e);
    int32_t rc = check_ready(e);
    if (rc) return rc;
    if (!all_ok) return B200_ERR_BAD_ARG;
    if (n_tuples == 0) { *all_ok = 1; return B200_SUCCESS; }
    if (!pk_offsets || !msgs32 || !sigs || n_tuples > kMaxBatchTuples) return B200_ERR_BAD_ARG;
    uint32_t nk;
    if ((rc = check_offsets(pk_offsets, n_tuples, &nk))) return rc;
    if (nk && !pks_flat) return B200_ERR_BAD_ARG;
    BlsState* s;
    rc = bls_state(e, &s);
    if (rc) return rc;
    const std::vector<uint32_t> moff = msg32_offsets(n_tuples);
    return verify_all(e, *s, {.keys = pks_flat, .n_keys = nk, .key_off = pk_offsets, .msgs = msgs32, .msg_off = moff.data(),
                              .n_msgs = uint32_t(n_tuples), .sigs = sigs, .T = uint32_t(n_tuples)}, seed32, 0, false, all_ok);
}

int32_t b200_fast_aggregate_verify_batch_indexed_all(const uint32_t* indices, const uint32_t* offsets, const uint8_t* msgs32,
                                                     const uint8_t* sigs, size_t n_tuples, const uint8_t* seed32, int32_t* all_ok) {
    Engine& e = engine();
    Guard g(e);
    int32_t rc = check_ready(e);
    if (rc) return rc;
    if (!all_ok) return B200_ERR_BAD_ARG;
    if (n_tuples == 0) { *all_ok = 1; return B200_SUCCESS; }
    if (!offsets || !msgs32 || !sigs || n_tuples > kMaxBatchTuples) return B200_ERR_BAD_ARG;
    BlsState* s;
    rc = bls_state(e, &s);
    if (rc) return rc;
    uint32_t ni;
    if ((rc = check_offsets(offsets, n_tuples, &ni))) return rc;
    if (ni && !indices) return B200_ERR_BAD_ARG;
    if ((rc = check_indices(e, *s, indices, ni, 0))) return rc;
    const std::vector<uint32_t> moff = msg32_offsets(n_tuples);
    static const uint32_t dummy = 0;
    return verify_all(e, *s, {.index = indices ? indices : &dummy, .n_index = ni, .key_off = offsets, .msgs = msgs32, .msg_off = moff.data(),
                              .n_msgs = uint32_t(n_tuples), .sigs = sigs, .T = uint32_t(n_tuples)}, seed32, 0, false, all_ok);
}

int32_t b200_fast_aggregate_verify_batch_all_sharded(const uint8_t* pks_flat, const uint32_t* pk_offsets, const uint8_t* msgs32,
                                                     const uint8_t* sigs, size_t n_tuples, const uint8_t seed32[32], int32_t* all_ok) {
    Engine& e = engine();
    Guard g(e);
    int32_t rc = check_ready(e);
    if (rc) return rc;
    const Comm& c = comm();
    if (!c.ready) { e.last_error = "b200_comm_init has not been called"; return B200_ERR_NOT_INITIALIZED; }
    if (!all_ok || !seed32) return B200_ERR_BAD_ARG;
    if (n_tuples == 0) { *all_ok = 1; return B200_SUCCESS; }
    if (!pk_offsets || !msgs32 || !sigs || n_tuples > kMaxBatchTuples) return B200_ERR_BAD_ARG;
    if (n_tuples < size_t(c.world)) { e.last_error = "fewer tuples than ranks"; return B200_ERR_BAD_ARG; }
    uint32_t nk;
    if ((rc = check_offsets(pk_offsets, n_tuples, &nk))) return rc;
    if (nk && !pks_flat) return B200_ERR_BAD_ARG;
    BlsState* s;
    rc = bls_state(e, &s);
    if (rc) return rc;
    const TupleRange mine = tuple_shard(n_tuples, size_t(c.world), size_t(c.rank));
    std::vector<uint32_t> koff, moff;
    return verify_all(e, *s, shard_batch(pks_flat, pk_offsets, msgs32, sigs, mine, koff, moff), seed32, uint64_t(mine.lo), true, all_ok);
}

int32_t b200_registry_load(const uint8_t* pks_flat, size_t n) {
    Engine& e = engine();
    Guard g(e);
    int32_t rc = check_ready(e);
    if (rc) return rc;
    if ((!pks_flat && n) || n > 0x7fffffffu) return B200_ERR_BAD_ARG;
    BlsState* s;
    rc = bls_state(e, &s);
    if (rc) return rc;
    B200_CUDA_TRY(s->keys.reserve(n * 48 + 64));
    B200_CUDA_TRY(s->reg_aff.reserve((n + kRegistryExtraKeys + 1) * sizeof(G1Aff)));
    B200_CUDA_TRY(s->reg_code.reserve((n + kRegistryExtraKeys + 1) * 4));
    if (n) B200_CUDA_TRY(cudaMemcpyAsync(s->keys.p, pks_flat, n * 48, cudaMemcpyHostToDevice, e.stream));
    B200_CUDA_TRY(cudaEventRecord(s->ev_k0, e.stream));
    launch_g1_validate(static_cast<const uint8_t*>(s->keys.p), uint32_t(n), static_cast<G1Aff*>(s->reg_aff.p),
                       static_cast<int32_t*>(s->reg_code.p), e.stream);
    e.launches += n ? 1 : 0;
    B200_CUDA_TRY(cudaEventRecord(s->ev_k1, e.stream));
    B200_CUDA_TRY(cudaGetLastError());
    B200_CUDA_TRY(cudaStreamSynchronize(e.stream));
    B200_CUDA_TRY(cudaEventElapsedTime(&e.last_kernel_ms, s->ev_k0, s->ev_k1));
    s->last_dominant_ms = e.last_kernel_ms;
    s->reg_n = n;
    return B200_SUCCESS;
}

int32_t b200_registry_key_codes(int32_t* out_codes, size_t n) {
    Engine& e = engine();
    Guard g(e);
    int32_t rc = check_ready(e);
    if (rc) return rc;
    BlsState* s;
    rc = bls_state(e, &s);
    if (rc) return rc;
    if (!out_codes || n > s->reg_n) return B200_ERR_BAD_ARG;
    if (n) B200_CUDA_TRY(cudaMemcpy(out_codes, s->reg_code.p, n * 4, cudaMemcpyDeviceToHost));
    return B200_SUCCESS;
}

static int32_t verify_batch_indexed(const uint8_t* extra_pks, size_t n_extra, const uint32_t* indices, const uint32_t* offsets,
                                    const uint8_t* msgs32, const uint8_t* sigs, size_t n_tuples, int32_t* out_codes) {
    Engine& e = engine();
    Guard g(e);
    int32_t rc = check_ready(e);
    if (rc) return rc;
    if (n_tuples == 0) return B200_SUCCESS;
    if (!offsets || !msgs32 || !sigs || !out_codes || n_tuples > kMaxBatchTuples) return B200_ERR_BAD_ARG;
    if ((n_extra && !extra_pks) || n_extra > kRegistryExtraKeys) return B200_ERR_BAD_ARG;
    BlsState* s;
    rc = bls_state(e, &s);
    if (rc) return rc;
    if (n_extra && !s->reg_aff.p) { e.last_error = "no registry loaded"; return B200_ERR_BAD_ARG; }
    uint32_t ni;
    if ((rc = check_offsets(offsets, n_tuples, &ni))) return rc;
    if (ni && !indices) return B200_ERR_BAD_ARG;
    if ((rc = check_indices(e, *s, indices, ni, n_extra))) return rc;
    const std::vector<uint32_t> moff = msg32_offsets(n_tuples);
    static const uint32_t dummy = 0;
    return run_verify(e, *s, {.keys = n_extra ? extra_pks : nullptr, .n_keys = uint32_t(n_extra), .index = indices ? indices : &dummy,
                              .n_index = ni, .key_off = offsets, .msgs = msgs32, .msg_off = moff.data(), .n_msgs = uint32_t(n_tuples),
                              .sigs = sigs, .T = uint32_t(n_tuples)}, out_codes);
}

int32_t b200_fast_aggregate_verify_batch_indexed(const uint32_t* indices, const uint32_t* offsets, const uint8_t* msgs32,
                                                 const uint8_t* sigs, size_t n_tuples, int32_t* out_codes) {
    return verify_batch_indexed(nullptr, 0, indices, offsets, msgs32, sigs, n_tuples, out_codes);
}

int32_t b200_fast_aggregate_verify_batch_mixed(const uint8_t* extra_pks, size_t n_extra, const uint32_t* indices,
                                               const uint32_t* offsets, const uint8_t* msgs32, const uint8_t* sigs,
                                               size_t n_tuples, int32_t* out_codes) {
    return verify_batch_indexed(extra_pks, n_extra, indices, offsets, msgs32, sigs, n_tuples, out_codes);
}

int32_t b200_fast_aggregate_verify(const uint8_t* const* pks, size_t k, const uint8_t* msg, size_t msg_len,
                                   const uint8_t sig[96]) {
    Engine& e = engine();
    Guard g(e);
    int32_t rc = check_ready(e);
    if (rc) return rc;
    if ((!pks && k) || (!msg && msg_len) || !sig || k > 0x7fffffffu || msg_len > 0x7fffffffu) return B200_ERR_BAD_ARG;
    BlsState* s;
    rc = bls_state(e, &s);
    if (rc) return rc;
    std::vector<uint8_t> flat(k * 48);
    for (size_t i = 0; i < k; i++) memcpy(flat.data() + 48 * i, pks[i], 48);
    const uint32_t koff[2] = {0, uint32_t(k)}, moff[2] = {0, uint32_t(msg_len)};
    int32_t code = B200_ERR_CUDA;
    rc = run_verify(e, *s, {.keys = flat.data(), .n_keys = uint32_t(k), .key_off = koff, .msgs = msg, .msg_off = moff, .n_msgs = 1,
                            .sigs = sig, .T = 1}, &code);
    return rc ? rc : code;
}

int32_t b200_eth_fast_aggregate_verify(const uint8_t* const* pks, size_t k, const uint8_t* msg, size_t msg_len,
                                       const uint8_t sig[96]) {
    if (k == 0 && sig) {
        bool inf = sig[0] == 0xc0;
        for (int i = 1; i < 96 && inf; i++) inf = sig[i] == 0;
        if (inf) return B200_SUCCESS;
    }
    return b200_fast_aggregate_verify(pks, k, msg, msg_len, sig);
}

int32_t b200_verify_signature(const uint8_t pk[48], const uint8_t* msg, size_t msg_len, const uint8_t sig[96]) {
    if (!pk) return B200_ERR_BAD_ARG;
    const uint8_t* one[1] = {pk};
    return b200_fast_aggregate_verify(one, 1, msg, msg_len, sig);
}

int32_t b200_aggregate_verify(const uint8_t* pks_flat, size_t n_pks, const uint8_t* const* msgs, const size_t* msg_lens,
                              size_t n_msgs, const uint8_t sig[96]) {
    Engine& e = engine();
    Guard g(e);
    int32_t rc = check_ready(e);
    if (rc) return rc;
    if ((!pks_flat && n_pks) || ((!msgs || !msg_lens) && n_msgs) || !sig || n_pks > 0x3fffffffu || n_msgs > 0x3fffffffu)
        return B200_ERR_BAD_ARG;
    BlsState* s;
    rc = bls_state(e, &s);
    if (rc) return rc;
    const bool shape_fail = (n_pks == 0 || n_pks != n_msgs);
    std::vector<uint32_t> moff(1, 0);
    std::vector<uint8_t> flat;
    if (!shape_fail) {
        size_t total = 0;
        for (size_t i = 0; i < n_msgs; i++) {
            if (msg_lens[i] > 0xffffffffu - total) { e.last_error = "aggregate_verify: messages exceed 4 GiB in total"; return B200_ERR_BAD_ARG; }
            total += msg_lens[i];
        }
        for (size_t i = 0; i < n_msgs; i++) {
            flat.insert(flat.end(), msgs[i], msgs[i] + msg_lens[i]);
            moff.push_back(uint32_t(flat.size()));
        }
    }
    int32_t code = B200_ERR_CUDA;
    rc = run_verify(e, *s, {.mode = MODE_AGGREGATE, .keys = pks_flat, .n_keys = uint32_t(n_pks), .msgs = flat.data(), .msg_off = moff.data(),
                            .n_msgs = uint32_t(moff.size() - 1), .sigs = sig, .T = 1, .force_fail_shape = shape_fail}, &code);
    return rc ? rc : code;
}

int32_t b200_aggregate(const uint8_t* sigs_flat, size_t n, uint8_t out[96]) {
    Engine& e = engine();
    Guard g(e);
    int32_t rc = check_ready(e);
    if (rc) return rc;
    if (n == 0) return B200_EMPTY_AGGREGATE;
    if (!sigs_flat || !out || n > 0x3fffffffu) return B200_ERR_BAD_ARG;
    BlsState* s;
    rc = bls_state(e, &s);
    if (rc) return rc;
    B200_CUDA_TRY(s->sigs.reserve(n * 96 + 64));
    B200_CUDA_TRY(s->g2pts.reserve((n + 1) * sizeof(G2Aff)));
    B200_CUDA_TRY(s->sig_code.reserve((n + 1) * 4));
    B200_CUDA_TRY(s->out.reserve(256));
    B200_CUDA_TRY(s->stage.reserve(256));
    cudaStream_t sa = e.stream;
    B200_CUDA_TRY(cudaMemcpyAsync(s->sigs.p, sigs_flat, n * 96, cudaMemcpyHostToDevice, sa));
    launch_g2_sig_decode(static_cast<const uint8_t*>(s->sigs.p), uint32_t(n), static_cast<G2Aff*>(s->g2pts.p),
                         static_cast<int32_t*>(s->sig_code.p), sa);
    uint8_t* d_out = static_cast<uint8_t*>(s->out.p);
    launch_g2_sum_compress(static_cast<const G2Aff*>(s->g2pts.p), static_cast<const int32_t*>(s->sig_code.p), uint32_t(n),
                           d_out + 16, reinterpret_cast<int32_t*>(d_out), sa);
    e.launches += 2;
    B200_CUDA_TRY(cudaGetLastError());
    B200_CUDA_TRY(cudaMemcpyAsync(s->stage.p, d_out, 16 + 96, cudaMemcpyDeviceToHost, sa));
    B200_CUDA_TRY(cudaStreamSynchronize(sa));
    const int32_t code = *static_cast<const int32_t*>(s->stage.p);
    if (code == B200_SUCCESS) memcpy(out, static_cast<const uint8_t*>(s->stage.p) + 16, 96);
    return code;
}

int32_t b200_eth_aggregate_public_keys(const uint8_t* pks_flat, size_t n, uint8_t out[48]) {
    Engine& e = engine();
    Guard g(e);
    int32_t rc = check_ready(e);
    if (rc) return rc;
    if (n == 0) return B200_EMPTY_AGGREGATE;
    if (!pks_flat || !out || n > 0x3fffffffu) return B200_ERR_BAD_ARG;
    BlsState* s;
    rc = bls_state(e, &s);
    if (rc) return rc;
    B200_CUDA_TRY(s->keys.reserve(n * 48 + 64));
    B200_CUDA_TRY(s->key_aff.reserve((n + 1) * sizeof(G1Aff)));
    B200_CUDA_TRY(s->key_code.reserve((n + 1) * 4));
    B200_CUDA_TRY(s->g1pts.reserve(2 * sizeof(G1Aff)));
    B200_CUDA_TRY(s->pk_code.reserve(16));
    B200_CUDA_TRY(s->flags.reserve(16));
    B200_CUDA_TRY(s->small.reserve(64));
    B200_CUDA_TRY(s->out.reserve(256));
    B200_CUDA_TRY(s->stage.reserve(256));
    cudaStream_t sa = e.stream;
    uint32_t* h = static_cast<uint32_t*>(s->stage.p);
    h[0] = 0; h[1] = uint32_t(n);
    B200_CUDA_TRY(cudaMemcpyAsync(s->small.p, h, 8, cudaMemcpyHostToDevice, sa));
    B200_CUDA_TRY(cudaMemcpyAsync(s->keys.p, pks_flat, n * 48, cudaMemcpyHostToDevice, sa));
    launch_g1_validate(static_cast<const uint8_t*>(s->keys.p), uint32_t(n), static_cast<G1Aff*>(s->key_aff.p),
                       static_cast<int32_t*>(s->key_code.p), sa);
    launch_g1_aggregate(static_cast<const G1Aff*>(s->key_aff.p), static_cast<const int32_t*>(s->key_code.p), nullptr,
                        static_cast<const uint32_t*>(s->small.p), 1, static_cast<G1Aff*>(s->g1pts.p), nullptr,
                        static_cast<int32_t*>(s->pk_code.p), static_cast<uint32_t*>(s->flags.p), 0u, sa);
    uint8_t* d_out = static_cast<uint8_t*>(s->out.p);
    launch_g1_compress(static_cast<const G1Aff*>(s->g1pts.p), d_out, sa);
    e.launches += 3;
    B200_CUDA_TRY(cudaGetLastError());
    B200_CUDA_TRY(cudaMemcpyAsync(h + 4, s->pk_code.p, 4, cudaMemcpyDeviceToHost, sa));
    B200_CUDA_TRY(cudaMemcpyAsync(h + 8, d_out, 48, cudaMemcpyDeviceToHost, sa));
    B200_CUDA_TRY(cudaStreamSynchronize(sa));
    const int32_t code = int32_t(h[4]);
    if (code == B200_SUCCESS) memcpy(out, h + 8, 48);
    return code;
}

}
```

ethereum_consensus_b200/csrc/pairing_vm.cuh:

```cuda
#pragma once
#include "fp12.cuh"
#include "pairing_vm_prog.cuh"
#include "pairing_vm_prog16.cuh"

namespace b200 {

enum VmOp : uint32_t { VM_NOP = 0, VM_MUL, VM_SQR, VM_MULFP, VM_INV, VM_ADD, VM_SUB, VM_NEG, VM_DBL, VM_CONJ, VM_MULXI, VM_COPY, VM_LDC };

struct VmRfDense {
    Fp2* p;
    B200_HD Fp2 load(uint32_t i) const { return p[i]; }
    B200_HD void store(uint32_t i, const Fp2& v) const { p[i] = v; }
};
#if !defined(B200_VM_SLOT_WORDS)
#define B200_VM_SLOT_WORDS 28
#endif
constexpr int kVmSlotWords = B200_VM_SLOT_WORDS;
#if defined(B200_VM_SLOT_PAD4)
B200_HD constexpr uint32_t vm_slot_word(uint32_t i) { return i * 24u + (i >> 2) * 4u; }
B200_HD constexpr uint32_t vm_team_words(uint32_t n_slots) { return n_slots * 24u + ((n_slots + 3u) >> 2) * 4u; }
#else
B200_HD constexpr uint32_t vm_slot_word(uint32_t i) { return i * uint32_t(kVmSlotWords); }
B200_HD constexpr uint32_t vm_team_words(uint32_t n_slots) { return n_slots * uint32_t(kVmSlotWords); }
#endif
constexpr int kVmMaxSmemBytes = 227 * 1024;
constexpr uint32_t kVmBlobMagic = 0xB200564Du;
struct VmRfStrided {
    uint32_t* p;
    B200_HD Fp2 load(uint32_t i) const {
        Fp2 v;
#if defined(__CUDA_ARCH__) && (B200_VM_SLOT_WORDS % 4 == 0)
        const uint4* q = reinterpret_cast<const uint4*>(p + vm_slot_word(i));
#pragma unroll
        for (int k = 0; k < 3; k++) {
            const uint4 a = q[k], b = q[3 + k];
            v.c0.l[4 * k] = a.x; v.c0.l[4 * k + 1] = a.y; v.c0.l[4 * k + 2] = a.z; v.c0.l[4 * k + 3] = a.w;
            v.c1.l[4 * k] = b.x; v.c1.l[4 * k + 1] = b.y; v.c1.l[4 * k + 2] = b.z; v.c1.l[4 * k + 3] = b.w;
        }
#else
        const uint32_t* q = p + vm_slot_word(i);
#pragma unroll
        for (int k = 0; k < 12; k++) { v.c0.l[k] = q[k]; v.c1.l[k] = q[12 + k]; }
#endif
        return v;
    }
    B200_HD void store(uint32_t i, const Fp2& v) const {
#if defined(__CUDA_ARCH__) && (B200_VM_SLOT_WORDS % 4 == 0)
        uint4* q = reinterpret_cast<uint4*>(p + vm_slot_word(i));
#pragma unroll
        for (int k = 0; k < 3; k++) {
            q[k] = make_uint4(v.c0.l[4 * k], v.c0.l[4 * k + 1], v.c0.l[4 * k + 2], v.c0.l[4 * k + 3]);
            q[3 + k] = make_uint4(v.c1.l[4 * k], v.c1.l[4 * k + 1], v.c1.l[4 * k + 2], v.c1.l[4 * k + 3]);
        }
#else
        uint32_t* q = p + vm_slot_word(i);
#pragma unroll
        for (int k = 0; k < 12; k++) { q[k] = v.c0.l[k]; q[12 + k] = v.c1.l[k]; }
#endif
    }
};

template <class RF>
B200_HD bool vm_exec(uint32_t w, const RF& rf, const Fp2* consts, Fp2& res) {
    const uint32_t op = w & 0xffu, a = (w >> 16) & 0xffu, b = w >> 24;
    switch (op) {
    case VM_NOP: return false;
    case VM_MUL: { const Fp2 x = rf.load(a), y = rf.load(b); fp2_mul(res, x, y); } break;
    case VM_SQR: { const Fp2 x = rf.load(a); fp2_sqr(res, x); } break;
    case VM_MULFP: { const Fp2 x = rf.load(a); const Fp k = rf.load(b).c0; fp2_mul_fp(res, x, k); } break;
    case VM_INV: { const Fp2 x = rf.load(a); fp2_inv(res, x); } break;
    case VM_ADD: { const Fp2 x = rf.load(a), y = rf.load(b); fp2_add(res, x, y); } break;
    case VM_SUB: { const Fp2 x = rf.load(a), y = rf.load(b); fp2_sub(res, x, y); } break;
    case VM_NEG: { const Fp2 x = rf.load(a); fp2_neg(res, x); } break;
    case VM_DBL: { const Fp2 x = rf.load(a); fp2_dbl(res, x); } break;
    case VM_CONJ: { const Fp2 x = rf.load(a); fp2_conj(res, x); } break;
    case VM_MULXI: { const Fp2 x = rf.load(a); fp2_mul_xi(res, x); } break;
    case VM_COPY: res = rf.load(a); break;
    default: res = consts[a]; break;
    }
    return true;
}

template <int TEAM> struct VmProg;
template <> struct VmProg<8> {
    static constexpr int team = 8, miller_rounds = kMillerRounds, miller_slots = kMillerSlots, final_rounds = kFinalRounds, final_slots = kFinalSlots;
    static constexpr const int* miller_out = kMillerOut;
    static constexpr const int* final_out = kFinalOut;
    static const uint32_t* miller_code() { return h_miller_code; }
    static const uint32_t* final_code() { return h_final_code; }
    static constexpr size_t miller_code_bytes = sizeof(h_miller_code), final_code_bytes = sizeof(h_final_code);
};
template <> struct VmProg<16> {
    static constexpr int team = 16, miller_rounds = kMillerRounds16, miller_slots = kMillerSlots16, final_rounds = kFinalRounds16, final_slots = kFinalSlots16;
    static constexpr const int* miller_out = kMillerOut16;
    static constexpr const int* final_out = kFinalOut16;
    static const uint32_t* miller_code() { return h_miller_code16; }
    static const uint32_t* final_code() { return h_final_code16; }
    static constexpr size_t miller_code_bytes = sizeof(h_miller_code16), final_code_bytes = sizeof(h_final_code16);
};

template <int TEAM>
inline void vm_run_host(const uint32_t* code, int n_rounds, const Fp2* consts, Fp2* rf_mem) {
    VmRfDense rf{rf_mem};
    for (int r = 0; r < n_rounds; r++) {
        Fp2 res[TEAM];
        bool live[TEAM];
        for (int l = 0; l < TEAM; l++) live[l] = vm_exec(code[r * TEAM + l], rf, consts, res[l]);
        for (int l = 0; l < TEAM; l++)
            if (live[l]) rf.store((code[r * TEAM + l] >> 8) & 0xffu, res[l]);
    }
}

B200_HD void vm_const_to_mont(Fp2& out, const uint32_t limbs[24]) {
    Fp a, b;
#pragma unroll
    for (int i = 0; i < 12; i++) { a.l[i] = limbs[i]; b.l[i] = limbs[12 + i]; }
    fp_to_mont(out.c0, a);
    fp_to_mont(out.c1, b);
}

}
```

Baseline: 34620.

## Fuse both pairings of each tuple into one shared-loop Miller program and single final exponentiation

Adds a generated fused VM program that evaluates the two Miller loops of a fast_aggregate_verify tuple together, so the f-squarings are shared, and writes one Fp12 per tuple. A single-input final exponentiation then replaces the two-input version. A 32-lane team variant is added for small batches. This removes one product of two Fp12 values per tuple and half of the squarings, at the cost of larger VM register files in shared memory and a build-time program generation step.

```diff
diff --git a/ethereum_consensus_b200/build.py b/ethereum_consensus_b200/build.py
--- a/ethereum_consensus_b200/build.py
+++ b/ethereum_consensus_b200/build.py
@@ -24,6 +24,17 @@
     return any(Path(d).stat().st_mtime > t for d in deps)
 
 
+GEN_VM = PKG.parent / "tools" / "gen_pairing_vm.py"
+FUSED_PROG = CSRC / "pairing_vm_fused_prog.cuh"
+
+
+def _fused_programs() -> None:
+    if _stale(FUSED_PROG, [GEN_VM, PKG.parent / "oracle" / "bls_oracle.py"]):
+        r = subprocess.run([sys.executable, str(GEN_VM), "--fused", str(FUSED_PROG)], capture_output=True, text=True)
+        if r.returncode != 0:
+            raise RuntimeError(f"pairing-VM program generation failed:\n{r.stdout}\n{r.stderr}")
+
+
 def build(force: bool = False, verbose: bool = False, defines=(), suffix: str = "", ptxas_opt=None) -> Path:
     global LIB, OBJ
     env_opt = {kv.split(":")[0]: int(kv.split(":")[1]) for kv in os.environ.get("B200_PTXAS_OPT", "").split(",") if kv}
@@ -31,6 +42,7 @@
     if suffix:
         LIB = PKG / f"libb200_consensus{suffix}.so"
         OBJ = PKG / f"build{suffix}"
+    _fused_programs()
     srcs = sorted(CSRC.glob("*.cu"))
     hdrs = sorted(CSRC.glob("*.cuh")) + sorted(CSRC.glob("*.h")) + sorted((PKG.parent / "include").glob("*.h"))
     OBJ.mkdir(exist_ok=True)
diff --git a/ethereum_consensus_b200/csrc/bls_kernels.cuh b/ethereum_consensus_b200/csrc/bls_kernels.cuh
--- a/ethereum_consensus_b200/csrc/bls_kernels.cuh
+++ b/ethereum_consensus_b200/csrc/bls_kernels.cuh
@@ -19,6 +19,7 @@
 void set_g1_small_n(uint32_t n);
 void set_small_cta(int threads);
 void set_vm_team16_max(uint32_t n);
+void set_vm_team32_max(uint32_t n);
 void set_vm_cta(int threads);
 void launch_g1_validate(const uint8_t* keys, uint32_t n, G1Aff* out, int32_t* codes, void* stream, int cta = 0);
 void launch_g1_aggregate(const G1Aff* keys, const int32_t* key_codes, const uint32_t* index, const uint32_t* off,
@@ -43,6 +44,10 @@
                       uint32_t n_pairs, Fp12* f, void* stream);
 void launch_vm_final(const Fp12* f, const uint32_t* pair_off, const int32_t* pk_code, const uint32_t* flags,
                      const int32_t* sig_code, uint32_t n_tuples, int32_t* out_codes, void* stream);
+void launch_vm_miller2(const G1Pre* g1, const uint32_t* g1_idx, const G2Aff* g2, const uint32_t* g2_idx, const int32_t* pk_code,
+                       const uint32_t* flags, const int32_t* sig_code, uint32_t n_tuples, Fp12* f, void* stream);
+void launch_vm_final1(const Fp12* f, const int32_t* pk_code, const uint32_t* flags, const int32_t* sig_code, uint32_t n_tuples,
+                      int32_t* out_codes, void* stream);
 void launch_g2_sum_compress(const G2Aff* sigs, const int32_t* sig_code, uint32_t n, uint8_t* out96, int32_t* out_code, void* stream);
 void launch_g1_compress(const G1Aff* p, uint8_t* out48, void* stream);
 void launch_neg_g1(G1Aff* out, G1Pre* out_pre, void* stream);
@@ -83,6 +88,10 @@
     PAIRING_EVAL_VM_MILLER8 = 32, PAIRING_EVAL_VM_MILLER16 = 33,
     PAIRING_EVAL_VM_FINAL8 = 34, PAIRING_EVAL_VM_FINAL16 = 35,
     PAIRING_EVAL_VM_END = 36,
+    PAIRING_EVAL_VM_MILLER2_8 = 40, PAIRING_EVAL_VM_MILLER2_16 = 41,
+    PAIRING_EVAL_VM_FINAL1_8 = 42, PAIRING_EVAL_VM_FINAL1_16 = 43,
+    PAIRING_EVAL_VM_MILLER2_32 = 44,
+    PAIRING_EVAL_VM2_END = 45,
     PAIRING_EVAL_FOLD_FP12 = 48, PAIRING_EVAL_FOLD_G2 = 49,
     PAIRING_EVAL_FOLD_END = 50
 };
@@ -92,5 +101,8 @@
                            Fp12* f, void* stream);
 void launch_vm_final_team(int team, const Fp12* f, const uint32_t* pair_off, const uint32_t* zeros, uint32_t n, Fp12* f_out,
                           int32_t* codes, void* stream);
+void launch_vm_miller2_team(int team, const G1Pre* g1, const uint32_t* idx, const G2Aff* g2, const uint32_t* zeros, uint32_t n_tuples,
+                            Fp12* f, void* stream);
+void launch_vm_final1_team(int team, const Fp12* f, const uint32_t* zeros, uint32_t n, Fp12* f_out, int32_t* codes, void* stream);
 
 }
diff --git a/ethereum_consensus_b200/csrc/bls_vm.cu b/ethereum_consensus_b200/csrc/bls_vm.cu
--- a/ethereum_consensus_b200/csrc/bls_vm.cu
+++ b/ethereum_consensus_b200/csrc/bls_vm.cu
@@ -26,7 +26,7 @@
 
 template <int TEAM>
 __device__ __forceinline__ void vm_run(const uint32_t* __restrict__ code, int n_rounds, const Fp2* __restrict__ consts,
-                                       const VmRfStrided& rf, uint32_t lane, bool active) {
+                                       const VmRfStrided& rf, uint32_t lane, bool active, uint32_t sync_mask = 0xffffffffu) {
     uint32_t w = __ldg(code + lane);
 #pragma unroll 1
     for (int r = 0; r < n_rounds; r++) {
@@ -36,7 +36,7 @@
             vm_exec(w, rf, consts, res);
             rf.store((w >> 8) & 0xffu, res);
         }
-        __syncwarp();
+        __syncwarp(sync_mask);
         w = w_next;
     }
 }
@@ -83,7 +83,53 @@
     }
 }
 
-template <int TEAM, bool STORE = false>
+template <int TEAM>
+__global__ void __launch_bounds__(128) k_vm_miller2(const uint32_t* __restrict__ code2, int rounds2, VmOuts outs2,
+                                                     const uint32_t* __restrict__ code1, int rounds1, VmOuts outs1,
+                                                     const Fp2* __restrict__ consts,
+                                                     const G1Pre* __restrict__ g1, const uint32_t* __restrict__ g1_idx,
+                                                     const G2Aff* __restrict__ g2, const uint32_t* __restrict__ g2_idx,
+                                                     const int32_t* __restrict__ pk_code, const uint32_t* __restrict__ flags,
+                                                     const int32_t* __restrict__ sig_code, uint32_t n_tuples,
+                                                     Fp12* __restrict__ f, int n_slots) {
+    extern __shared__ uint32_t smem[];
+    const uint32_t team_in_block = threadIdx.x / TEAM, lane = threadIdx.x % TEAM;
+    const uint32_t t = blockIdx.x * (blockDim.x / TEAM) + team_in_block;
+    const uint32_t team_mask = (TEAM == 32 ? 0xffffffffu : ((1u << TEAM) - 1u)) << ((threadIdx.x % 32u) & ~uint32_t(TEAM - 1));
+    VmRfStrided rf{smem + team_in_block * vm_team_words(uint32_t(n_slots))};
+    const bool active = t < n_tuples && !tuple_dead(t, pk_code, flags, sig_code);
+    const G1Pre* p[2] = {nullptr, nullptr};
+    const G2Aff* q[2] = {nullptr, nullptr};
+    int n_live = 0;
+    if (active) {
+#pragma unroll
+        for (int k = 0; k < 2; k++) {
+            const G1Pre* pk = g1 + g1_idx[2 * t + k];
+            const G2Aff* qk = g2 + g2_idx[2 * t + k];
+            if (!(pk->inf || qk->inf)) { p[n_live] = pk; q[n_live] = qk; n_live++; }
+        }
+        for (uint32_t k = lane; k < 5u * uint32_t(n_live); k += TEAM) {
+            const uint32_t j = k / 5u, c = k % 5u;
+            Fp2 v;
+            if (c < 3) { v.c0 = c == 0 ? p[j]->xz : (c == 1 ? p[j]->y : p[j]->z3); v.c1 = fp_zero(); }
+            else v = c == 3 ? q[j]->x : q[j]->y;
+            rf.store(k, v);
+        }
+    }
+    __syncwarp(team_mask);
+    const bool fused = n_live == 2;
+    vm_run<TEAM>(fused ? code2 : code1, n_live == 0 ? 0 : (fused ? rounds2 : rounds1), consts, rf, lane, true, team_mask);
+    static_assert(TEAM >= 6, "team must cover the six output coefficients");
+    if (active && lane < 6) {
+        Fp2 v;
+        if (n_live == 0) v = (lane == 0) ? fp2_one() : fp2_zero();
+        else v = rf.load(uint32_t(fused ? outs2.v[lane] : outs1.v[lane]));
+        const int tower_pos[6] = {0, 3, 1, 4, 2, 5};
+        reinterpret_cast<Fp2*>(f + t)[tower_pos[lane]] = v;
+    }
+}
+
+template <int TEAM, int NF, bool STORE = false>
 __global__ void __launch_bounds__(128) k_vm_final(const uint32_t* __restrict__ code, const Fp2* __restrict__ consts,
                                                   const Fp12* __restrict__ f, const uint32_t* __restrict__ pair_off,
                                                   const int32_t* __restrict__ pk_code, const uint32_t* __restrict__ flags,
@@ -104,8 +150,9 @@
     }
     if (active) {
         const int tower_pos[6] = {0, 3, 1, 4, 2, 5};
-        for (uint32_t k = lane; k < 12; k += TEAM) {
-            const Fp2* src = reinterpret_cast<const Fp2*>(f + pair_off[t] + k / 6);
+        const Fp12* fs = NF == 2 ? f + pair_off[t] : f + t;
+        for (uint32_t k = lane; k < 6 * NF; k += TEAM) {
+            const Fp2* src = reinterpret_cast<const Fp2*>(fs + k / 6);
             rf.store(k, src[tower_pos[k % 6]]);
         }
     }
@@ -133,11 +180,14 @@
     int rounds = 0, slots = 0;
     VmOuts outs{};
 };
-static VmProgramDev g_miller_prog[2], g_final_prog[2];
+static VmProgramDev g_miller_prog[3], g_final_prog[3];
+static VmProgramDev g_miller2_prog[3], g_final1_prog[3];
 static Fp2* g_d_consts = nullptr;
 static uint32_t g_team16_max = 2048;
+static uint32_t g_team32_max = 256;
 static int g_vm_cta = 32;
 void set_vm_team16_max(uint32_t n) { g_team16_max = n; }
+void set_vm_team32_max(uint32_t n) { g_team32_max = n; }
 void set_vm_cta(int threads) { if (threads == 32 || threads == 64 || threads == 128) g_vm_cta = threads; }
 
 static int vm_set_program(VmProgramDev& p, const uint32_t* code, size_t bytes, int rounds, int slots, const int* outs, cudaStream_t st) {
@@ -154,10 +204,17 @@
 static int vm_upload(int slot, cudaStream_t st) {
     typedef VmProg<TEAM> P;
     if (vm_set_program(g_miller_prog[slot], P::miller_code(), P::miller_code_bytes, P::miller_rounds, P::miller_slots, P::miller_out, st)) return 1;
-    if (vm_set_program(g_final_prog[slot], P::final_code(), P::final_code_bytes, P::final_rounds, P::final_slots, P::final_out, st)) return 1;
-    cudaFuncSetAttribute(k_vm_miller<TEAM>, cudaFuncAttributeMaxDynamicSharedMemorySize, kVmMaxSmemBytes);
-    cudaFuncSetAttribute(k_vm_final<TEAM>, cudaFuncAttributeMaxDynamicSharedMemorySize, kVmMaxSmemBytes);
-    cudaFuncSetAttribute(k_vm_final<TEAM, true>, cudaFuncAttributeMaxDynamicSharedMemorySize, kVmMaxSmemBytes);
+    if (vm_set_program(g_miller2_prog[slot], P::miller2_code(), P::miller2_code_bytes, P::miller2_rounds, P::miller2_slots, P::miller2_out, st)) return 1;
+    cudaFuncSetAttribute(k_vm_miller2<TEAM>, cudaFuncAttributeMaxDynamicSharedMemorySize, kVmMaxSmemBytes);
+    if constexpr (TEAM != 32) {
+        if (vm_set_program(g_final_prog[slot], P::final_code(), P::final_code_bytes, P::final_rounds, P::final_slots, P::final_out, st)) return 1;
+        if (vm_set_program(g_final1_prog[slot], P::final1_code(), P::final1_code_bytes, P::final1_rounds, P::final1_slots, P::final1_out, st)) return 1;
+        cudaFuncSetAttribute(k_vm_miller<TEAM>, cudaFuncAttributeMaxDynamicSharedMemorySize, kVmMaxSmemBytes);
+        cudaFuncSetAttribute(k_vm_final<TEAM, 2>, cudaFuncAttributeMaxDynamicSharedMemorySize, kVmMaxSmemBytes);
+        cudaFuncSetAttribute(k_vm_final<TEAM, 2, true>, cudaFuncAttributeMaxDynamicSharedMemorySize, kVmMaxSmemBytes);
+        cudaFuncSetAttribute(k_vm_final<TEAM, 1>, cudaFuncAttributeMaxDynamicSharedMemorySize, kVmMaxSmemBytes);
+        cudaFuncSetAttribute(k_vm_final<TEAM, 1, true>, cudaFuncAttributeMaxDynamicSharedMemorySize, kVmMaxSmemBytes);
+    }
     return 0;
 }
 
@@ -198,7 +255,7 @@
     if (g_d_consts) return 0;
     cudaStream_t st = static_cast<cudaStream_t>(stream);
     uint32_t* d_plain = nullptr;
-    if (vm_upload<8>(0, st) || vm_upload<16>(1, st)) return 1;
+    if (vm_upload<8>(0, st) || vm_upload<16>(1, st) || vm_upload<32>(2, st)) return 1;
     if (cudaMalloc(&g_d_consts, sizeof(Fp2) * kVmConsts) != cudaSuccess) return 1;
     if (cudaMalloc(&d_plain, sizeof(h_vm_consts)) != cudaSuccess) return 1;
     cudaMemcpyAsync(d_plain, h_vm_consts, sizeof(h_vm_consts), cudaMemcpyHostToDevice, st);
@@ -220,16 +277,31 @@
     k_vm_miller<TEAM><<<(n_pairs + teams - 1) / teams, threads, smem, st>>>(
         p.d_code, g_d_consts, g1, g1_idx, g2, g2_idx, pair_tuple, pk_code, flags, sig_code, n_pairs, f, p.rounds, p.slots, p.outs);
 }
-template <int TEAM, bool STORE = false>
+template <int TEAM>
+static void launch_vm_miller2_t(int slot, const G1Pre* g1, const uint32_t* g1_idx, const G2Aff* g2, const uint32_t* g2_idx,
+                                const int32_t* pk_code, const uint32_t* flags, const int32_t* sig_code, uint32_t n_tuples, Fp12* f,
+                                cudaStream_t st) {
+    const VmProgramDev& p2 = g_miller2_prog[slot];
+    const VmProgramDev& p1 = g_miller_prog[slot];
+    const int slots = std::max(p2.slots, p1.slots);
+    int threads = g_vm_cta;
+    while (threads > 32 && size_t(threads / TEAM) * vm_team_words(uint32_t(slots)) * 4 > size_t(kVmMaxSmemBytes)) threads >>= 1;
+    const int teams = threads / TEAM;
+    const size_t smem = size_t(teams) * vm_team_words(uint32_t(slots)) * 4;
+    k_vm_miller2<TEAM><<<(n_tuples + teams - 1) / teams, threads, smem, st>>>(
+        p2.d_code, p2.rounds, p2.outs, p1.d_code, p1.rounds, p1.outs, g_d_consts, g1, g1_idx, g2, g2_idx, pk_code, flags, sig_code,
+        n_tuples, f, slots);
+}
+template <int TEAM, int NF, bool STORE = false>
 static void launch_vm_final_t(int slot, const Fp12* f, const uint32_t* pair_off, const int32_t* pk_code, const uint32_t* flags,
                               const int32_t* sig_code, uint32_t n_tuples, int32_t* out_codes, cudaStream_t st,
                               Fp12* f_out = nullptr) {
-    const VmProgramDev& p = g_final_prog[slot];
+    const VmProgramDev& p = NF == 2 ? g_final_prog[slot] : g_final1_prog[slot];
     int threads = g_vm_cta;
     while (threads > 32 && size_t(threads / TEAM) * vm_team_words(uint32_t(p.slots)) * 4 > size_t(kVmMaxSmemBytes)) threads >>= 1;
     const int teams = threads / TEAM;
     const size_t smem = size_t(teams) * vm_team_words(uint32_t(p.slots)) * 4;
-    k_vm_final<TEAM, STORE><<<(n_tuples + teams - 1) / teams, threads, smem, st>>>(
+    k_vm_final<TEAM, NF, STORE><<<(n_tuples + teams - 1) / teams, threads, smem, st>>>(
         p.d_code, g_d_consts, f, pair_off, pk_code, flags, sig_code, n_tuples, out_codes, p.rounds, p.slots, p.outs, f_out);
 }
 
@@ -245,8 +317,23 @@
                      const int32_t* sig_code, uint32_t n_tuples, int32_t* out_codes, void* stream) {
     if (!n_tuples) return;
     cudaStream_t st = static_cast<cudaStream_t>(stream);
-    if (n_tuples <= g_team16_max) launch_vm_final_t<16>(1, f, pair_off, pk_code, flags, sig_code, n_tuples, out_codes, st);
-    else launch_vm_final_t<8>(0, f, pair_off, pk_code, flags, sig_code, n_tuples, out_codes, st);
+    if (n_tuples <= g_team16_max) launch_vm_final_t<16, 2>(1, f, pair_off, pk_code, flags, sig_code, n_tuples, out_codes, st);
+    else launch_vm_final_t<8, 2>(0, f, pair_off, pk_code, flags, sig_code, n_tuples, out_codes, st);
+}
+void launch_vm_miller2(const G1Pre* g1, const uint32_t* g1_idx, const G2Aff* g2, const uint32_t* g2_idx, const int32_t* pk_code,
+                       const uint32_t* flags, const int32_t* sig_code, uint32_t n_tuples, Fp12* f, void* stream) {
+    if (!n_tuples) return;
+    cudaStream_t st = static_cast<cudaStream_t>(stream);
+    if (n_tuples <= g_team32_max) launch_vm_miller2_t<32>(2, g1, g1_idx, g2, g2_idx, pk_code, flags, sig_code, n_tuples, f, st);
+    else if (n_tuples <= g_team16_max) launch_vm_miller2_t<16>(1, g1, g1_idx, g2, g2_idx, pk_code, flags, sig_code, n_tuples, f, st);
+    else launch_vm_miller2_t<8>(0, g1, g1_idx, g2, g2_idx, pk_code, flags, sig_code, n_tuples, f, st);
+}
+void launch_vm_final1(const Fp12* f, const int32_t* pk_code, const uint32_t* flags, const int32_t* sig_code, uint32_t n_tuples,
+                      int32_t* out_codes, void* stream) {
+    if (!n_tuples) return;
+    cudaStream_t st = static_cast<cudaStream_t>(stream);
+    if (n_tuples <= g_team16_max) launch_vm_final_t<16, 1>(1, f, nullptr, pk_code, flags, sig_code, n_tuples, out_codes, st);
+    else launch_vm_final_t<8, 1>(0, f, nullptr, pk_code, flags, sig_code, n_tuples, out_codes, st);
 }
 
 void launch_vm_miller_team(int team, const G1Pre* g1, const uint32_t* idx, const G2Aff* g2, const uint32_t* zeros, uint32_t n,
@@ -262,8 +349,24 @@
     if (!n) return;
     cudaStream_t st = static_cast<cudaStream_t>(stream);
     const int32_t* z = reinterpret_cast<const int32_t*>(zeros);
-    if (team == 16) launch_vm_final_t<16, true>(1, f, pair_off, z, zeros, z, n, codes, st, f_out);
-    else launch_vm_final_t<8, true>(0, f, pair_off, z, zeros, z, n, codes, st, f_out);
-}
-
-}
+    if (team == 16) launch_vm_final_t<16, 2, true>(1, f, pair_off, z, zeros, z, n, codes, st, f_out);
+    else launch_vm_final_t<8, 2, true>(0, f, pair_off, z, zeros, z, n, codes, st, f_out);
+}
+void launch_vm_miller2_team(int team, const G1Pre* g1, const uint32_t* idx, const G2Aff* g2, const uint32_t* zeros, uint32_t n_tuples,
+                            Fp12* f, void* stream) {
+    if (!n_tuples) return;
+    cudaStream_t st = static_cast<cudaStream_t>(stream);
+    const int32_t* z = reinterpret_cast<const int32_t*>(zeros);
+    if (team == 32) launch_vm_miller2_t<32>(2, g1, idx, g2, idx, z, zeros, z, n_tuples, f, st);
+    else if (team == 16) launch_vm_miller2_t<16>(1, g1, idx, g2, idx, z, zeros, z, n_tuples, f, st);
+    else launch_vm_miller2_t<8>(0, g1, idx, g2, idx, z, zeros, z, n_tuples, f, st);
+}
+void launch_vm_final1_team(int team, const Fp12* f, const uint32_t* zeros, uint32_t n, Fp12* f_out, int32_t* codes, void* stream) {
+    if (!n) return;
+    cudaStream_t st = static_cast<cudaStream_t>(stream);
+    const int32_t* z = reinterpret_cast<const int32_t*>(zeros);
+    if (team == 16) launch_vm_final_t<16, 1, true>(1, f, nullptr, z, zeros, z, n, codes, st, f_out);
+    else launch_vm_final_t<8, 1, true>(0, f, nullptr, z, zeros, z, n, codes, st, f_out);
+}
+
+}
diff --git a/ethereum_consensus_b200/csrc/capi_bls.cu b/ethereum_consensus_b200/csrc/capi_bls.cu
--- a/ethereum_consensus_b200/csrc/capi_bls.cu
+++ b/ethereum_consensus_b200/csrc/capi_bls.cu
@@ -62,6 +62,7 @@
     {"bls_k1_first_cta", [](BlsState& s, int64_t v) { s.k1_first_cta = (v == 128) ? 128 : 384; }},
     {"bls_small_cta", [](BlsState& s, int64_t v) { s.small_cta_override = int(v); }},
     {"vm_team16_max", [](BlsState&, int64_t v) { set_vm_team16_max(uint32_t(std::max<int64_t>(0, v))); }},
+    {"vm_team32_max", [](BlsState&, int64_t v) { set_vm_team32_max(uint32_t(std::max<int64_t>(0, v))); }},
     {"vm_cta", [](BlsState&, int64_t v) { set_vm_cta(int(v)); }},
 };
 
@@ -322,10 +323,9 @@
         B200_CUDA_TRY(cudaStreamWaitEvent(sd, s.ev_ck[c], 0));
         launch_g1_aggregate(static_cast<const G1Aff*>(s.key_aff.p), static_cast<const int32_t*>(s.key_code.p), nullptr, d_small + o_koff + t0,
                             nt, nullptr, static_cast<G1Pre*>(s.g1pre.p) + t0, d_pk + t0, d_fl + t0, 0u, sd, nullptr);
-        launch_vm_miller(static_cast<const G1Pre*>(s.g1pre.p), d_g1i + 2 * t0, static_cast<const G2Aff*>(s.g2pts.p), d_g2i + 2 * t0,
-                         d_ptu + 2 * t0, d_pk, d_fl, d_sc, 2 * nt, static_cast<Fp12*>(s.f.p) + 2 * size_t(t0), sd);
-        launch_vm_final(static_cast<const Fp12*>(s.f.p), d_poff + t0, d_pk + t0, d_fl + t0, d_sc + t0, nt,
-                        static_cast<int32_t*>(s.out.p) + t0, sd);
+        launch_vm_miller2(static_cast<const G1Pre*>(s.g1pre.p), d_g1i + 2 * t0, static_cast<const G2Aff*>(s.g2pts.p), d_g2i + 2 * t0,
+                          d_pk + t0, d_fl + t0, d_sc + t0, nt, static_cast<Fp12*>(s.f.p) + t0, sd);
+        launch_vm_final1(static_cast<const Fp12*>(s.f.p) + t0, d_pk + t0, d_fl + t0, d_sc + t0, nt, static_cast<int32_t*>(s.out.p) + t0, sd);
         e.launches += 3;
     }
     B200_CUDA_TRY(cudaEventRecord(s.ev_join, sd));
@@ -402,9 +402,9 @@
     const uint32_t* d_fl = static_cast<const uint32_t*>(s.flags.p);
     const int32_t* d_sc = static_cast<const int32_t*>(s.sig_code.p);
     if (fa && s.use_vm) {
-        launch_vm_miller(static_cast<const G1Pre*>(s.g1pre.p), d_g1i, d_g2, d_g2i, d_ptu, d_pk, d_fl, d_sc, n_pairs, static_cast<Fp12*>(s.f.p), sa);
+        launch_vm_miller2(static_cast<const G1Pre*>(s.g1pre.p), d_g1i, d_g2, d_g2i, d_pk, d_fl, d_sc, T, static_cast<Fp12*>(s.f.p), sa);
         if (s.trace) cudaEventRecord(s.ev_t[3], sa);
-        launch_vm_final(static_cast<const Fp12*>(s.f.p), d_poff, d_pk, d_fl, d_sc, T, static_cast<int32_t*>(s.out.p), sa);
+        launch_vm_final1(static_cast<const Fp12*>(s.f.p), d_pk, d_fl, d_sc, T, static_cast<int32_t*>(s.out.p), sa);
     } else {
         const G1Aff* pair_g1 = static_cast<const G1Aff*>(fa ? s.g1pts.p : s.key_aff.p);
         launch_miller(pair_g1, d_g1i, d_g2, d_g2i, d_ptu, d_pk, d_fl, d_sc, n_pairs, static_cast<Fp12*>(s.f.p), sa);
@@ -697,7 +697,7 @@
     Guard g(e);
     int32_t rc = check_ready(e);
     if (rc) return rc;
-    const bool vm = op >= PAIRING_EVAL_VM_MILLER8 && op < PAIRING_EVAL_VM_END;
+    const bool vm = (op >= PAIRING_EVAL_VM_MILLER8 && op < PAIRING_EVAL_VM_END) || (op >= PAIRING_EVAL_VM_MILLER2_8 && op < PAIRING_EVAL_VM2_END);
     const bool fold = op >= PAIRING_EVAL_FOLD_FP12 && op < PAIRING_EVAL_FOLD_END;
     if (!(vm || fold || (op >= 0 && op < PAIRING_EVAL_END)) || n > (1u << 24)) return B200_ERR_BAD_ARG;
     if (n == 0) return B200_SUCCESS;
@@ -708,7 +708,10 @@
     const size_t rec_bytes = size_t(n) * W * 4;
     cudaStream_t st = e.stream;
     std::vector<uint32_t> h_out(size_t(n) * W, 0);
-    const int team = (op == PAIRING_EVAL_VM_MILLER16 || op == PAIRING_EVAL_VM_FINAL16) ? 16 : 8;
+    const int team = op == PAIRING_EVAL_VM_MILLER2_32 ? 32 : (op == PAIRING_EVAL_VM_MILLER16 || op == PAIRING_EVAL_VM_FINAL16 ||
+                                                             op == PAIRING_EVAL_VM_MILLER2_16 || op == PAIRING_EVAL_VM_FINAL1_16) ? 16 : 8;
+    const bool pair2 = op == PAIRING_EVAL_VM_MILLER2_8 || op == PAIRING_EVAL_VM_MILLER2_16 || op == PAIRING_EVAL_VM_MILLER2_32;
+    if (pair2 && (n & 1u)) return B200_ERR_BAD_ARG;
     uint8_t* d = nullptr;
     const size_t scratch = 3 * rec_bytes + size_t(n) * (sizeof(Fp12) * 3 + sizeof(G2Jac) + sizeof(G1Pre) + sizeof(G2Aff) + 12) + 4096;
     B200_CUDA_TRY(cudaMalloc(&d, scratch));
@@ -731,7 +734,7 @@
         ce = cudaGetLastError();
         if (ce == cudaSuccess) ce = cudaMemcpyAsync(h_out.data(), dout, rec_bytes, cudaMemcpyDeviceToHost, st);
         if (ce == cudaSuccess) ce = cudaStreamSynchronize(st);
-    } else if (op == PAIRING_EVAL_VM_MILLER8 || op == PAIRING_EVAL_VM_MILLER16) {
+    } else if (op == PAIRING_EVAL_VM_MILLER8 || op == PAIRING_EVAL_VM_MILLER16 || pair2) {
         std::vector<G1Pre> g1(n);
         std::vector<G2Aff> g2(n);
         std::vector<uint32_t> idx(n);
@@ -750,12 +753,32 @@
         cudaMemcpyAsync(dg2, g2.data(), n * sizeof(G2Aff), cudaMemcpyHostToDevice, st);
         cudaMemcpyAsync(didx, idx.data(), n * 4, cudaMemcpyHostToDevice, st);
         cudaMemsetAsync(dzero, 0, n * 4, st);
-        launch_vm_miller_team(team, dg1, didx, dg2, dzero, n, df, st);
+        const uint32_t n_f = pair2 ? n / 2 : n;
+        if (pair2) launch_vm_miller2_team(team, dg1, didx, dg2, dzero, n_f, df, st);
+        else launch_vm_miller_team(team, dg1, didx, dg2, dzero, n, df, st);
         e.launches++;
         ce = cudaGetLastError();
-        if (ce == cudaSuccess) ce = cudaMemcpyAsync(f.data(), df, n * sizeof(Fp12), cudaMemcpyDeviceToHost, st);
+        if (ce == cudaSuccess) ce = cudaMemcpyAsync(f.data(), df, n_f * sizeof(Fp12), cudaMemcpyDeviceToHost, st);
         if (ce == cudaSuccess) ce = cudaStreamSynchronize(st);
-        for (uint32_t i = 0; i < n; i++) put(i, &f[i], sizeof(Fp12), 0);
+        for (uint32_t i = 0; i < n_f; i++) put(i, &f[i], sizeof(Fp12), 0);
+    } else if (op == PAIRING_EVAL_VM_FINAL1_8 || op == PAIRING_EVAL_VM_FINAL1_16) {
+        std::vector<Fp12> f(n);
+        for (uint32_t i = 0; i < n; i++) f[i] = fp12_of(a + i * W);
+        Fp12* df = reinterpret_cast<Fp12*>(carve(n * sizeof(Fp12)));
+        Fp12* dfo = reinterpret_cast<Fp12*>(carve(n * sizeof(Fp12)));
+        uint32_t* dzero = reinterpret_cast<uint32_t*>(carve(n * 4));
+        int32_t* dcodes = reinterpret_cast<int32_t*>(carve(n * 4));
+        std::vector<Fp12> fo(n);
+        std::vector<int32_t> codes(n);
+        cudaMemcpyAsync(df, f.data(), n * sizeof(Fp12), cudaMemcpyHostToDevice, st);
+        cudaMemsetAsync(dzero, 0, n * 4, st);
+        launch_vm_final1_team(team, df, dzero, n, dfo, dcodes, st);
+        e.launches++;
+        ce = cudaGetLastError();
+        if (ce == cudaSuccess) ce = cudaMemcpyAsync(fo.data(), dfo, n * sizeof(Fp12), cudaMemcpyDeviceToHost, st);
+        if (ce == cudaSuccess) ce = cudaMemcpyAsync(codes.data(), dcodes, n * 4, cudaMemcpyDeviceToHost, st);
+        if (ce == cudaSuccess) ce = cudaStreamSynchronize(st);
+        for (uint32_t i = 0; i < n; i++) put(i, &fo[i], sizeof(Fp12), codes[i] == BLS_SUCCESS ? 1u : 0u);
     } else if (vm) {
         std::vector<Fp12> f(2 * size_t(n));
         std::vector<uint32_t> off(n);
diff --git a/ethereum_consensus_b200/csrc/pairing_vm.cuh b/ethereum_consensus_b200/csrc/pairing_vm.cuh
--- a/ethereum_consensus_b200/csrc/pairing_vm.cuh
+++ b/ethereum_consensus_b200/csrc/pairing_vm.cuh
@@ -2,6 +2,7 @@
 #include "fp12.cuh"
 #include "pairing_vm_prog.cuh"
 #include "pairing_vm_prog16.cuh"
+#include "pairing_vm_fused_prog.cuh"
 
 namespace b200 {
 
@@ -89,6 +90,12 @@
     static const uint32_t* miller_code() { return h_miller_code; }
     static const uint32_t* final_code() { return h_final_code; }
     static constexpr size_t miller_code_bytes = sizeof(h_miller_code), final_code_bytes = sizeof(h_final_code);
+    static constexpr int miller2_rounds = kMiller2Rounds, miller2_slots = kMiller2Slots, final1_rounds = kFinal1Rounds, final1_slots = kFinal1Slots;
+    static constexpr const int* miller2_out = kMiller2Out;
+    static constexpr const int* final1_out = kFinal1Out;
+    static const uint32_t* miller2_code() { return h_miller2_code; }
+    static const uint32_t* final1_code() { return h_final1_code; }
+    static constexpr size_t miller2_code_bytes = sizeof(h_miller2_code), final1_code_bytes = sizeof(h_final1_code);
 };
 template <> struct VmProg<16> {
     static constexpr int team = 16, miller_rounds = kMillerRounds16, miller_slots = kMillerSlots16, final_rounds = kFinalRounds16, final_slots = kFinalSlots16;
@@ -97,6 +104,22 @@
     static const uint32_t* miller_code() { return h_miller_code16; }
     static const uint32_t* final_code() { return h_final_code16; }
     static constexpr size_t miller_code_bytes = sizeof(h_miller_code16), final_code_bytes = sizeof(h_final_code16);
+    static constexpr int miller2_rounds = kMiller2Rounds16, miller2_slots = kMiller2Slots16, final1_rounds = kFinal1Rounds16, final1_slots = kFinal1Slots16;
+    static constexpr const int* miller2_out = kMiller2Out16;
+    static constexpr const int* final1_out = kFinal1Out16;
+    static const uint32_t* miller2_code() { return h_miller2_code16; }
+    static const uint32_t* final1_code() { return h_final1_code16; }
+    static constexpr size_t miller2_code_bytes = sizeof(h_miller2_code16), final1_code_bytes = sizeof(h_final1_code16);
+};
+template <> struct VmProg<32> {
+    static constexpr int team = 32, miller_rounds = kMillerRounds32, miller_slots = kMillerSlots32;
+    static constexpr const int* miller_out = kMillerOut32;
+    static const uint32_t* miller_code() { return h_miller_code32; }
+    static constexpr size_t miller_code_bytes = sizeof(h_miller_code32);
+    static constexpr int miller2_rounds = kMiller2Rounds32, miller2_slots = kMiller2Slots32;
+    static constexpr const int* miller2_out = kMiller2Out32;
+    static const uint32_t* miller2_code() { return h_miller2_code32; }
+    static constexpr size_t miller2_code_bytes = sizeof(h_miller2_code32);
 };
 
 template <int TEAM>
```

After: 35080 (median of 6 runs). 1.01x the previous value.
